# dwkim606/optimal_conv

Measured on AMD Instinct MI355X. Metric: homomorphic convs/sec (conv_then_pack + BN bias, k x k, batch B, N=2^16), higher is better.
Workload: dtype u64; 1 GPU; conv 3 3; ker_wid=3, batch=256, in_wid=16, logN=16, moduli=ckks.DefaultBootstrapParams[6] Q0,Q1 + P=0x1fffffffffe00001, ciphertexts_per_launch_set=4, contexts_per_gpu=4, chunk_nodes=512

## Files before the change

### optimal_conv_amd/csrc/hc_arith.h

```cpp
#pragma once
#include <stdint.h>

#if defined(__HIPCC__) || defined(HC_EMU)
#define HC_HD __host__ __device__ __forceinline__
#else
#define HC_HD inline
#endif

typedef uint64_t u64;
typedef unsigned int u32;
typedef unsigned __int128 u128;

HC_HD u64 hc_mulhi(u64 a, u64 b) {
#if defined(__HIP_DEVICE_COMPILE__)
    return __umul64hi(a, b);
#else
    return (u64)(((u128)a * b) >> 64);
#endif
}

HC_HD u64 hc_mul_shoup_lazy(u64 x, u64 w, u64 wp, u64 q) {
    u64 hi = hc_mulhi(x, wp);
    return x * w - hi * q;
}
HC_HD double hc_f64_mulmod(double x, double w, double wq, double q) {
#pragma clang fp contract(off)
    const double h = x * w;
    const double l = __builtin_fma(x, w, -h);
    const double k = __builtin_rint(x * wq);
    const double r = __builtin_fma(-k, q, h);
    return r + l;
}
HC_HD double hc_f64_reduce(double u, double q, double qinv) {
#pragma clang fp contract(off)
    return __builtin_fma(-__builtin_rint(u * qinv), q, u);
}
HC_HD double hc_u2d(u64 x) { return __builtin_bit_cast(double, x); }
HC_HD u64 hc_d2u(double x) { return __builtin_bit_cast(u64, x); }
HC_HD double hc_f64_from_u(u64 x) { return hc_u2d(x | 0x4330000000000000ull) - 4503599627370496.0; }
HC_HD u64 hc_f64_to_u_plus(double v, u64 base) { return (hc_d2u(v + 6755399441055744.0) & 0x000FFFFFFFFFFFFFull) + (base - 0x0008000000000000ull); }

HC_HD u64 hc_shoup_companion(u64 w, u64 q) {
    u64 r = w, quo = 0;
    for (int i = 0; i < 64; i++) {
        r <<= 1; quo <<= 1;
        if (r >= q) { r -= q; quo |= 1; }
    }
    return quo;
}
HC_HD u64 hc_csub(u64 x, u64 q) { return x >= q ? x - q : x; }

HC_HD u64 hc_mulhi_lo2(u64 x, u64 p) {
    const u32 x0 = (u32)x, x1 = (u32)(x >> 32), p0 = (u32)p, p1 = (u32)(p >> 32);
    return (u64)x1 * p1 + (((u64)x0 * p1) >> 32) + (((u64)x1 * p0) >> 32);
}
HC_HD u64 hc_opaque_uniform(u64 v) {
#if defined(__HIP_DEVICE_COMPILE__)
    u64 r;
    asm("; uniform constant kept opaque" : "=s"(r) : "0"(v));
    return r;
#else
    return v;
#endif
}
struct HcQ { u64 q, nq, q4, nq4, nq2; };
HC_HD HcQ hc_q(u64 q) {
    HcQ Q; Q.q = q; Q.nq = hc_opaque_uniform(0 - q); Q.q4 = 4 * q; Q.nq4 = hc_opaque_uniform(0 - 4 * q); Q.nq2 = hc_opaque_uniform(0 - 2 * q);
    return Q;
}
HC_HD u64 hc_shoup4(u64 x, u64 w, u64 wp, const HcQ &Q) { return x * w + hc_mulhi_lo2(x, wp) * Q.nq; }
HC_HD u64 hc_fold(u64 x, u64 nb) { const u64 t = x + nb; return (int)(u32)(t >> 32) < 0 ? x : t; }
HC_HD u64 hc_canon4(u64 x, const HcQ &Q) { return hc_fold(hc_fold(x, Q.nq2), Q.nq); }
HC_HD u64 hc_canon8(u64 x, const HcQ &Q) { return hc_canon4(hc_fold(x, Q.nq4), Q); }
HC_HD u64 hc_reduce64(u64 x, u64 mu, const HcQ &Q) { return hc_canon4(x + hc_mulhi_lo2(x, mu) * Q.nq, Q); }
HC_HD u64 hc_mul_shoup(u64 x, u64 w, u64 wp, u64 q) { return hc_csub(hc_mul_shoup_lazy(x, w, wp, q), q); }

HC_HD u64 hc_mont(u64 a, u64 b, u64 q, u64 qinv) {
    u128 m = (u128)a * b;
    u64 lo = (u64)m, hi = (u64)(m >> 64);
    u64 h = hc_mulhi(lo * qinv, q);
    u64 r = hi - h;
    return hi < h ? r + q : r;
}
HC_HD u64 hc_mont_redc(u128 T, u64 q, u64 qinv) {
    const u64 lo = (u64)T, hi = (u64)(T >> 64);
    const u64 h = hc_mulhi(lo * qinv, q);
    const u64 r = hi - h;
    return hi < h ? r + q : r;
}
HC_HD u64 hc_addmod(u64 a, u64 b, u64 q) { return hc_csub(a + b, q); }
HC_HD u64 hc_submod(u64 a, u64 b, u64 q) { return a >= b ? a - b : a + q - b; }

struct HcMod {
    u64 q;
    u64 qinv;
    u64 r2;
    u64 ninv, ninv_s;
    u64 mu;
    u64 row32;
};
```

### optimal_conv_amd/csrc/hc_kernels.h

```cpp
#pragma once
#include "hc_arith.h"

#define HC_TPB 256
#ifndef HC_MIN_WAVES
#define HC_MIN_WAVES 4
#endif
#define HC_ROWS_LDS 4096
#define HC_COLS_LDS 4096

struct __attribute__((aligned(16))) HcTw { u64 w, ws; };

#define HC_SMALL_Q(q) ((q) < (1ull << 31))
template <bool B> struct HcBool { static constexpr bool value = B; };
template <int V> struct HcInt { static constexpr int value = V; };
#define HC_COUNT_DISPATCH(n, body) do { switch (n) { case 1: body(HcInt<1>{}); break; case 2: body(HcInt<2>{}); break; case 3: body(HcInt<3>{}); break; case 4: body(HcInt<4>{}); break; \
    case 5: body(HcInt<5>{}); break; case 6: body(HcInt<6>{}); break; case 7: body(HcInt<7>{}); break; case 8: body(HcInt<8>{}); break; default: break; } } while (0)
#define HC_LD(S32, rowptr, j) ((S32) ? hc_ld32(rowptr, j) : (rowptr)[j])
#define HC_ST(S32, rowptr, j, v) do { if (S32) hc_st32(rowptr, j, v); else (rowptr)[j] = (v); } while (0)
#define HC_ROW_DISPATCH(row32, body) do { if (row32) body(HcBool<true>{}); else body(HcBool<false>{}); } while (0)
__device__ __forceinline__ u64 hc_ld32(const u64 *row, size_t j) { return (u64)reinterpret_cast<const u32 *>(row)[j]; }
__device__ __forceinline__ void hc_st32(u64 *row, size_t j, u64 v) { reinterpret_cast<u32 *>(row)[j] = (u32)v; }
struct __attribute__((packed, aligned(4))) HcU64A4 { u64 v; };
__device__ __forceinline__ u64 hc_ldp(const u64 *row, size_t j, bool row32) {
    return reinterpret_cast<const HcU64A4 *>(reinterpret_cast<const char *>(row) + (j << (row32 ? 2 : 3)))->v & (row32 ? 0xFFFFFFFFull : ~0ull);
}
struct HcTwTab {
    const HcTw *rowsA;
    const HcTw *rowsB;
    const HcTw *colsA;
    const HcTw *colsB;
    HcTw ninv;
    HcTw w_last_ninv;
};

struct __attribute__((aligned(8))) HcTw32 { u32 w, ws; };
struct HcTwTab32 { const HcTw32 *rowsA, *rowsB, *colsA, *colsB; };

enum { HC_FM_FREE = 1, HC_FM_ALT = 2 };
template <int FM, class TW>
__device__ __forceinline__ void hc_ct_round(u64 (&e)[16], const TW &tw, const HcQ &Q) {
#pragma unroll
    for (int s = 0; s < 4; s++) {
        const int half = 8 >> s;
#pragma unroll
        for (int g = 0; g < (1 << s); g++) {
            const HcTw w = tw((1 << s) - 1 + g);
#pragma unroll
            for (int k = 0; k < half; k++) {
                const int a = g * 2 * half + k, b = a + half;
                u64 X = e[a];
                if (FM == HC_FM_ALT) X = hc_fold(X, Q.nq4);
                const u64 T = hc_shoup4(e[b], w.w, w.ws, Q);
                e[a] = X + T;
                e[b] = (X + Q.q4) - T;
            }
        }
    }
}
template <int FM>
__device__ __forceinline__ u64 hc_fwd_canon(u64 x, const HcQ &Q, u64 mu) {
    if (FM == HC_FM_FREE) return hc_reduce64(x, mu, Q);
    return hc_canon8(x, Q);
}
template <bool LAST, class TW>
__device__ __forceinline__ void hc_gs_round(u64 (&e)[16], const TW &tw, const HcQ &Q, HcTw ninv, HcTw w_last) {
#pragma unroll
    for (int s = 0; s < 4; s++) {
        const int dist = 1 << s;
#pragma unroll
        for (int g = 0; g < (8 >> s); g++) {
            HcTw w = tw((8 >> s) - 1 + g);
            if (LAST && s == 3) w = w_last;
#pragma unroll
            for (int k = 0; k < dist; k++) {
                const int a = g * 2 * dist + k, b = a + dist;
                const u64 X = e[a], Y = e[b], u = X + Y, d = (X + Q.q4) - Y;
                if (LAST && s == 3) e[a] = hc_shoup4(u, ninv.w, ninv.ws, Q);
                else e[a] = hc_fold(u, Q.nq4);
                e[b] = hc_shoup4(d, w.w, w.ws, Q);
            }
        }
    }
}

struct HcF64Mod { double q, qinv; };
template <bool LAST, class TW>
__device__ __forceinline__ void hc_gs_round_f64(double (&e)[16], const TW &tw, HcF64Mod m, HcTw ninv, HcTw w_last) {
#pragma unroll
    for (int s = 0; s < 4; s++) {
        const int dist = 1 << s;
#pragma unroll
        for (int g = 0; g < (8 >> s); g++) {
            HcTw w = tw((8 >> s) - 1 + g);
            if (LAST && s == 3) w = w_last;
            const double ww = hc_u2d(w.w), wq = hc_u2d(w.ws);
#pragma unroll
            for (int k = 0; k < dist; k++) {
                const int a = g * 2 * dist + k, b = a + dist;
                const double X = e[a], Y = e[b], u = X + Y, d = X - Y;
                if (LAST && s == 3) e[a] = hc_f64_mulmod(u, hc_u2d(ninv.w), hc_u2d(ninv.ws), m.q);
                else e[a] = (s & 1) ? hc_f64_reduce(u, m.q, m.qinv) : u;
                e[b] = hc_f64_mulmod(d, ww, wq, m.q);
            }
        }
    }
}

#ifndef HC_ROWS_WAVE_SYNC
#define HC_ROWS_WAVE_SYNC 1
#endif
#if defined(HC_EMU) || !HC_ROWS_WAVE_SYNC
#define HC_ROW_SYNC() __syncthreads()
#else
#define HC_ROW_SYNC() do { __builtin_amdgcn_fence(__ATOMIC_RELEASE, "wavefront"); __builtin_amdgcn_wave_barrier(); __builtin_amdgcn_fence(__ATOMIC_ACQUIRE, "wavefront"); } while (0)
#endif
__device__ __forceinline__ int hc_rows_lds(int rloc, int col) {
    return rloc * 256 + ((col & 0xF0) ^ ((rloc & 1) << 4)) + ((col & 15) ^ ((col >> 5) & 7) ^ ((rloc & 1) << 3));
}
__device__ __forceinline__ int hc_cols_lds(int row, int c) { return ((row ^ ((row >> 4) & 1)) << 4) + c; }

#if defined(__HIP_DEVICE_COMPILE__)
typedef const HcTw __attribute__((address_space(1))) *HcTwGlobalPtr;
typedef const HcTw __attribute__((address_space(4))) *HcTwConstPtr;
#define HC_TW_LOAD(p, i) (*((HcTwGlobalPtr)(p) + (i)))
#define HC_TW_LOADK(p, i) (*((HcTwConstPtr)(p) + (i)))
#else
#define HC_TW_LOAD(p, i) ((p)[i])
#define HC_TW_LOADK(p, i) ((p)[i])
#endif
template <class T>
__device__ __forceinline__ T hc_const_copy(const T *p) {
    T r;
#if defined(__HIP_DEVICE_COMPILE__)
    static_assert(sizeof(T) % 8 == 0 && alignof(T) >= 8, "hc_const_copy: whole 8-byte words");
    typedef const u64 __attribute__((address_space(4))) *W;
    const W src = (W)(const void *)p; u64 *dst = reinterpret_cast<u64 *>(&r);
#pragma unroll
    for (unsigned i = 0; i < sizeof(T) / 8; i++) dst[i] = src[i];
#else
    r = *p;
#endif
    return r;
}
template <bool KC = false> struct HcRowsTwA { const HcTw *p; __device__ __forceinline__ HcTw operator()(int slot) const { if (KC) return HC_TW_LOADK(p, slot); else return HC_TW_LOAD(p, slot); } };
#ifndef HC_DBG_TWB_FIXED
#define HC_DBG_TWB_FIXED 0
#endif
template <bool KC = false> struct HcRowsTwB { const HcTw *p; __device__ __forceinline__ HcTw operator()(int slot) const { if (HC_DBG_TWB_FIXED) slot = 0; if (KC) return HC_TW_LOADK(p, slot * 16); else return HC_TW_LOAD(p, slot * 16); } };

template <int FM, bool KC = false>
__device__ __forceinline__ void hc_rows_fwd(u64 (&e)[16], u64 *lds, const HcTwTab &T, int row, int rloc, int tid, const HcQ &Q) {
    hc_ct_round<FM>(e, HcRowsTwA<KC>{T.rowsA + row * 16}, Q);
#pragma unroll
    for (int hi = 0; hi < 16; hi++) lds[hc_rows_lds(rloc, hi * 16 + tid)] = e[hi];
    HC_ROW_SYNC();
#pragma unroll
    for (int lo = 0; lo < 16; lo++) e[lo] = lds[hc_rows_lds(rloc, tid * 16 + lo)];
    hc_ct_round<FM>(e, HcRowsTwB<KC>{T.rowsB + row * 256 + tid}, Q);
}
template <bool KC = false>
__device__ __forceinline__ void hc_rows_inv(u64 (&e)[16], u64 *lds, const HcTwTab &T, int row, int rloc, int tid, const HcQ &Q) {
    hc_gs_round<false>(e, HcRowsTwB<KC>{T.rowsB + row * 256 + tid}, Q, T.ninv, T.ninv);
#pragma unroll
    for (int lo = 0; lo < 16; lo++) lds[hc_rows_lds(rloc, tid * 16 + lo)] = e[lo];
    HC_ROW_SYNC();
#pragma unroll
    for (int hi = 0; hi < 16; hi++) e[hi] = lds[hc_rows_lds(rloc, hi * 16 + tid)];
    hc_gs_round<false>(e, HcRowsTwA<KC>{T.rowsA + row * 16}, Q, T.ninv, T.ninv);
}
template <int FM, bool KC = false>
__device__ __forceinline__ void hc_cols_fwd(u64 (&e)[16], u64 *lds, const HcTwTab &T, int c, int tid, const HcQ &Q) {
    hc_ct_round<FM>(e, HcRowsTwA<KC>{T.colsA}, Q);
#pragma unroll
    for (int hi = 0; hi < 16; hi++) lds[hc_cols_lds(hi * 16 + tid, c)] = e[hi];
    __syncthreads();
#pragma unroll
    for (int lo = 0; lo < 16; lo++) e[lo] = lds[hc_cols_lds(tid * 16 + lo, c)];
    hc_ct_round<FM>(e, HcRowsTwB<KC>{T.colsB + tid}, Q);
}
template <bool SCALE = true, bool KC = false>
__device__ __forceinline__ void hc_cols_inv(u64 (&e)[16], u64 *lds, const HcTwTab &T, int c, int tid, const HcQ &Q) {
    hc_gs_round<false>(e, HcRowsTwB<KC>{T.colsB + tid}, Q, T.ninv, T.ninv);
#pragma unroll
    for (int lo = 0; lo < 16; lo++) lds[hc_cols_lds(tid * 16 + lo, c)] = e[lo];
    __syncthreads();
#pragma unroll
    for (int hi = 0; hi < 16; hi++) e[hi] = lds[hc_cols_lds(hi * 16 + tid, c)];
    hc_gs_round<SCALE>(e, HcRowsTwA<KC>{T.colsA}, Q, T.ninv, T.w_last_ninv);
}

__device__ __forceinline__ void hc_rows_inv_f64(double (&e)[16], u64 *lds, const HcTwTab &T, int row, int rloc, int tid, HcF64Mod m) {
    hc_gs_round_f64<false>(e, HcRowsTwB<false>{T.rowsB + row * 256 + tid}, m, T.ninv, T.ninv);
#pragma unroll
    for (int lo = 0; lo < 16; lo++) lds[hc_rows_lds(rloc, tid * 16 + lo)] = hc_d2u(e[lo]);
    HC_ROW_SYNC();
#pragma unroll
    for (int hi = 0; hi < 16; hi++) e[hi] = hc_u2d(lds[hc_rows_lds(rloc, hi * 16 + tid)]);
    hc_gs_round_f64<false>(e, HcRowsTwA<false>{T.rowsA + row * 16}, m, T.ninv, T.ninv);
}
__device__ __forceinline__ void hc_cols_inv_f64(double (&e)[16], u64 *lds, const HcTwTab &T, int c, int tid, HcF64Mod m) {
    hc_gs_round_f64<false>(e, HcRowsTwB<false>{T.colsB + tid}, m, T.ninv, T.ninv);
#pragma unroll
    for (int lo = 0; lo < 16; lo++) lds[hc_cols_lds(tid * 16 + lo, c)] = hc_d2u(e[lo]);
    __syncthreads();
#pragma unroll
    for (int hi = 0; hi < 16; hi++) e[hi] = hc_u2d(lds[hc_cols_lds(hi * 16 + tid, c)]);
    hc_gs_round_f64<true>(e, HcRowsTwA<false>{T.colsA}, m, T.ninv, T.w_last_ninv);
}

__device__ __forceinline__ void hc_rows_lin_to_lo(u64 (&e)[16], u64 *lds, int t, int rloc, int tid) {
#pragma unroll
    for (int k = 0; k < 16; k++) lds[hc_rows_lds(k, t)] = e[k];
    __syncthreads();
#pragma unroll
    for (int lo = 0; lo < 16; lo++) e[lo] = lds[hc_rows_lds(rloc, tid * 16 + lo)];
}
__device__ __forceinline__ void hc_rows_lo_to_lin(u64 (&e)[16], u64 *lds, int t, int rloc, int tid) {
#pragma unroll
    for (int lo = 0; lo < 16; lo++) lds[hc_rows_lds(rloc, tid * 16 + lo)] = e[lo];
    __syncthreads();
#pragma unroll
    for (int k = 0; k < 16; k++) e[k] = lds[hc_rows_lds(k, t)];
}

#ifndef HC_MM_LDS32
#define HC_MM_LDS32 1
#endif
#ifndef HC_MM_WAVES
#define HC_MM_WAVES 7
#endif
#ifndef HC_MM_WAVES_EXT
#define HC_MM_WAVES_EXT 5
#endif
#ifndef HC_CV_LDS32
#define HC_CV_LDS32 1
#endif
#if HC_CV_LDS32
typedef u32 hc_cvc_lds_t;
#else
typedef u64 hc_cvc_lds_t;
#endif
typedef u64 hc_cvr_lds_t;
#if HC_MM_LDS32
typedef u32 hc_mm_lds_t;
#else
typedef u64 hc_mm_lds_t;
#endif
__device__ __forceinline__ int hc_rows_lds32(int rloc, int col) {
    return rloc * 256 + ((col & 0xF0) ^ ((rloc & 1) << 4) ^ ((rloc & 2) << 4)) + ((col & 15) ^ ((col >> 5) & 7) ^ ((rloc & 1) << 3));
}
__device__ __forceinline__ int hc_cols_lds32(int row, int c) { return ((row ^ ((row >> 4) & 3)) << 4) + c; }
template <class WA, class RA, class SY>
__device__ __forceinline__ void hc_xchg32(u64 (&e)[16], u32 *lds, WA wa, RA ra, SY sync) {
    u32 lo[16];
#pragma unroll
    for (int i = 0; i < 16; i++) lds[wa(i)] = (u32)e[i];
    sync();
#pragma unroll
    for (int i = 0; i < 16; i++) lo[i] = lds[ra(i)];
    sync();
#pragma unroll
    for (int i = 0; i < 16; i++) lds[wa(i)] = (u32)(e[i] >> 32);
    sync();
#pragma unroll
    for (int i = 0; i < 16; i++) e[i] = ((u64)lds[ra(i)] << 32) | lo[i];
}
template <int FM, bool KC = false>
__device__ __forceinline__ void hc_rows_fwd(u64 (&e)[16], u32 *lds, const HcTwTab &T, int row, int rloc, int tid, const HcQ &Q) {
    hc_ct_round<FM>(e, HcRowsTwA<KC>{T.rowsA + row * 16}, Q);
    hc_xchg32(e, lds, [&](int hi) { return hc_rows_lds32(rloc, hi * 16 + tid); }, [&](int lo) { return hc_rows_lds32(rloc, tid * 16 + lo); }, [] { HC_ROW_SYNC(); });
    hc_ct_round<FM>(e, HcRowsTwB<KC>{T.rowsB + row * 256 + tid}, Q);
}
template <bool KC = false>
__device__ __forceinline__ void hc_rows_inv(u64 (&e)[16], u32 *lds, const HcTwTab &T, int row, int rloc, int tid, const HcQ &Q) {
    hc_gs_round<false>(e, HcRowsTwB<KC>{T.rowsB + row * 256 + tid}, Q, T.ninv, T.ninv);
    hc_xchg32(e, lds, [&](int lo) { return hc_rows_lds32(rloc, tid * 16 + lo); }, [&](int hi) { return hc_rows_lds32(rloc, hi * 16 + tid); }, [] { HC_ROW_SYNC(); });
    hc_gs_round<false>(e, HcRowsTwA<KC>{T.rowsA + row * 16}, Q, T.ninv, T.ninv);
}
template <int FM, bool KC = false>
__device__ __forceinline__ void hc_cols_fwd(u64 (&e)[16], u32 *lds, const HcTwTab &T, int c, int tid, const HcQ &Q) {
    hc_ct_round<FM>(e, HcRowsTwA<KC>{T.colsA}, Q);
    hc_xchg32(e, lds, [&](int hi) { return hc_cols_lds32(hi * 16 + tid, c); }, [&](int lo) { return hc_cols_lds32(tid * 16 + lo, c); }, [] { __syncthreads(); });
    hc_ct_round<FM>(e, HcRowsTwB<KC>{T.colsB + tid}, Q);
}
template <bool SCALE = true, bool KC = false>
__device__ __forceinline__ void hc_cols_inv(u64 (&e)[16], u32 *lds, const HcTwTab &T, int c, int tid, const HcQ &Q) {
    hc_gs_round<false>(e, HcRowsTwB<KC>{T.colsB + tid}, Q, T.ninv, T.ninv);
    hc_xchg32(e, lds, [&](int lo) { return hc_cols_lds32(tid * 16 + lo, c); }, [&](int hi) { return hc_cols_lds32(hi * 16 + tid, c); }, [] { __syncthreads(); });
    hc_gs_round<SCALE>(e, HcRowsTwA<KC>{T.colsA}, Q, T.ninv, T.w_last_ninv);
}
template <class WA, class RA, class SY>
__device__ __forceinline__ void hc_xchg32_f64(double (&f)[16], u32 *lds, WA wa, RA ra, SY sync) {
    u64 b[16];
#pragma unroll
    for (int i = 0; i < 16; i++) b[i] = hc_d2u(f[i]);
    hc_xchg32(b, lds, wa, ra, sync);
#pragma unroll
    for (int i = 0; i < 16; i++) f[i] = hc_u2d(b[i]);
}
// ... 390 lines not shown
#define HC_JOB_FAST 0
#endif
#if HC_JOB_FAST
#define HC_JOB blockIdx.x
#define HC_TILE blockIdx.y
#define HC_NJOBS gridDim.x
#else
#define HC_JOB blockIdx.y
#define HC_TILE blockIdx.x
#define HC_NJOBS gridDim.y
#endif
#define HC_FREE_OFF 72
#ifndef HC_W_A1
#define HC_W_A1 4
#endif
#ifndef HC_W_A2
#define HC_W_A2 4
#endif
#ifndef HC_W_A3
#define HC_W_A3 4
#endif
#ifndef HC_W_B1
#define HC_W_B1 4
#endif
#ifndef HC_W_B2
#define HC_W_B2 1
#endif
#ifndef HC_W_B3
#define HC_W_B3 4
#endif
#ifndef HC_W_B4
#define HC_W_B4 1
#endif
struct HcLoopA {
    const HcTw *ctc;
    HcPtrs ker;
    u64 *tmp;
    u64 *cts;
    int i0, norm;
    int slot0, slot_step;
    size_t cts_stride;
    int njobs;
    HcMod m0, m1;
    HcTw q1inv;
    u64 h, negh0;
};
#ifndef HC_A_WAVES
#define HC_A_WAVES 4
#endif
template <int F64>
__global__ __launch_bounds__(HC_TPB, HC_W_A1) void hc_k_a1(HcLoopA A, HcTwTab T1inv) {
    __shared__ hc_cvr_lds_t lds[HC_ROWS_LDS];
    const int t = threadIdx.x, tid = t & 15, rloc = t >> 4, row = HC_TILE * 16 + rloc;
    const int job = HC_JOB, p = job & 1, i = A.i0 + (job >> 1) * A.norm, z = blockIdx.z;
    const HcTw *__restrict__ c = A.ctc + ((size_t)z * 4 + (size_t)p * 2 + 1) * 65536;
    const u64 *__restrict__ k = A.ker.p[z] + ((size_t)i * 2 + 1) * 65536;
    const HcQ Q = hc_q(A.m1.q);
    u64 e[16];
#pragma unroll
    for (int kk = 0; kk < 16; kk++) {
        const size_t off = (size_t)(HC_TILE * 16 + kk) * 256 + t;
        const HcTw cw = c[off];
        e[kk] = hc_shoup4(k[off], cw.w, cw.ws, Q);
    }
    u64 *o = A.tmp + ((size_t)z * A.njobs + job) * 65536 + (size_t)row * 256;
    hc_rows_lin_to_lo(e, lds, t, rloc, tid);
    HC_ROW_SYNC();
    if (F64) {
        const HcF64Mod m{(double)A.m1.q, 1.0 / (double)A.m1.q};
        double f[16];
#pragma unroll
        for (int kk = 0; kk < 16; kk++) f[kk] = hc_f64_reduce(hc_f64_from_u(e[kk]), m.q, m.qinv);
        hc_rows_inv_f64(f, lds, T1inv, row, rloc, tid, m);
#pragma unroll
        for (int hi = 0; hi < 16; hi++) o[hi * 16 + tid] = hc_d2u(f[hi]);
    } else {
        hc_rows_inv(e, lds, T1inv, row, rloc, tid, Q);
#pragma unroll
        for (int hi = 0; hi < 16; hi++) o[hi * 16 + tid] = e[hi];
    }
}
template <int FM, int F64>
__global__ __launch_bounds__(HC_TPB, HC_W_A2) void hc_k_a2(HcLoopA A, HcTwTab T1inv, HcTwTab T0fwd) {
    __shared__ hc_cvc_lds_t lds[HC_COLS_LDS];
    const int t = threadIdx.x, c = t & 15, tid = t >> 4;
    u64 *base = A.tmp + (size_t)HC_JOB * 65536 + HC_TILE * 16 + c;
    const HcQ Q0 = hc_q(A.m0.q);
    u64 e[16];
#pragma unroll
    for (int lo = 0; lo < 16; lo++) e[lo] = base[(size_t)(tid * 16 + lo) * 256];
    if (F64) {
        const double q1 = (double)A.m1.q, hh = (double)A.h;
        const HcF64Mod m{q1, 1.0 / q1};
        double f[16];
#pragma unroll
        for (int lo = 0; lo < 16; lo++) f[lo] = hc_u2d(e[lo]);
        hc_cols_inv_f64(f, lds, T1inv, c, tid, m);
#pragma unroll
        for (int hi = 0; hi < 16; hi++) {
            double v = f[hi];
            v = v > hh ? v - q1 : (v < -hh ? v + q1 : v);
            e[hi] = hc_f64_to_u_plus(v, A.m0.q);
        }
    } else {
        const HcQ Q1 = hc_q(A.m1.q);
        hc_cols_inv(e, lds, T1inv, c, tid, Q1);
#pragma unroll
        for (int hi = 0; hi < 16; hi++) {
            const u64 v = hc_csub(hc_canon4(e[hi], Q1) + A.h, A.m1.q);
            e[hi] = hc_reduce64(v + A.negh0, A.m0.mu, Q0);
        }
    }
    __syncthreads();
    hc_cols_fwd<FM>(e, lds, T0fwd, c, tid, Q0);
#pragma unroll
    for (int lo = 0; lo < 16; lo++) base[(size_t)(tid * 16 + lo) * 256] = e[lo];
}
template <int FM>
__global__ __launch_bounds__(HC_TPB, HC_W_A3) void hc_k_a3(HcLoopA A, HcTwTab T0fwd) {
    __shared__ hc_cvr_lds_t lds[HC_ROWS_LDS];
    const int t = threadIdx.x, tid = t & 15, rloc = t >> 4, row = HC_TILE * 16 + rloc;
    const int job = HC_JOB, p = job & 1, i = A.i0 + (job >> 1) * A.norm, z = blockIdx.z;
    const u64 *__restrict__ in = A.tmp + ((size_t)z * A.njobs + job) * 65536 + (size_t)row * 256;
    const HcTw *__restrict__ c = A.ctc + ((size_t)z * 4 + (size_t)p * 2) * 65536 + (size_t)HC_TILE * 4096 + t;
    const u64 *__restrict__ k = A.ker.p[z] + ((size_t)i * 2) * 65536 + (size_t)HC_TILE * 4096 + t;
    u64 *__restrict__ o = A.cts + (size_t)z * A.cts_stride + ((size_t)(A.slot0 + (job >> 1) * A.slot_step) * 2 + p) * 65536 + (size_t)HC_TILE * 4096 + t;
    const HcQ Q = hc_q(A.m0.q);
    u64 e[16], a0[16];
#pragma unroll
    for (int hi = 0; hi < 16; hi++) e[hi] = in[hi * 16 + tid];
#pragma unroll
    for (int kk = 0; kk < 16; kk++) a0[kk] = k[kk * 256];
#pragma unroll
    for (int kk = 0; kk < 16; kk++) { const HcTw cw = c[kk * 256]; a0[kk] = hc_shoup4(a0[kk], cw.w, cw.ws, Q); }
    hc_rows_fwd<FM>(e, lds, T0fwd, row, rloc, tid, Q);
    HC_ROW_SYNC();
    hc_rows_lo_to_lin(e, lds, t, rloc, tid);
#pragma unroll
    for (int kk = 0; kk < 16; kk++) {
        const u64 d = FM == HC_FM_FREE ? a0[kk] + HC_FREE_OFF * Q.q - e[kk] : a0[kk] + Q.q - hc_canon8(e[kk], Q);
        o[kk * 256] = hc_canon4(hc_shoup4(d, A.q1inv.w, A.q1inv.ws, Q), Q);
    }
}

struct HcLoopB {
    const u64 *src;
    u64 *dst;
    u64 *tmpC;
    u64 *tmpE;
    u64 *tmpT;
    const HcTw *idx;
    const HcTw *evkQ;
    const HcTw *evkP;
    int n0, step, norm;
    int nodes;
    size_t src_stride, dst_stride;
    HcMod m0, mp;
    HcTw pmodq;
    HcTw pinv;
    u64 mu0;
    u64 vthresh;
    u32 gal;
};
__global__ __launch_bounds__(HC_TPB, HC_W_B1) void hc_k_b1(HcLoopB B, HcTwTab T0inv) {
    __shared__ hc_cvr_lds_t lds[HC_ROWS_LDS];
    const int t = threadIdx.x, tid = t & 15, rloc = t >> 4, row = HC_TILE * 16 + rloc;
    const int job = HC_JOB, z = job / B.nodes, node = job - z * B.nodes, i = (B.n0 + node) * B.norm;
    const size_t tile = (size_t)HC_TILE * 4096 + t;
    const u64 *__restrict__ y1 = B.src + (size_t)z * B.src_stride + ((size_t)i * 2 + 1) * 65536 + tile;
    const u64 *__restrict__ x1 = B.src + (size_t)z * B.src_stride + ((size_t)(i + B.step) * 2 + 1) * 65536 + tile;
    const HcTw *__restrict__ idx = B.idx + tile;
    const HcQ Q = hc_q(B.m0.q);
    u64 e[16], yy[16];
#pragma unroll
    for (int kk = 0; kk < 16; kk++) { e[kk] = x1[kk * 256]; yy[kk] = y1[kk * 256]; }
#pragma unroll
    for (int kk = 0; kk < 16; kk++) {
        const HcTw I = idx[kk * 256];
        e[kk] = hc_fold(yy[kk] + Q.q4 - hc_shoup4(e[kk], I.w, I.ws, Q), Q.nq4);
    }
    if (B.tmpT != nullptr) {
        u64 *__restrict__ tt = B.tmpT + (size_t)job * 65536 + tile;
#pragma unroll
        for (int kk = 0; kk < 16; kk++) tt[kk * 256] = e[kk];
    }
    hc_rows_lin_to_lo(e, lds, t, rloc, tid);
    HC_ROW_SYNC();
    hc_rows_inv(e, lds, T0inv, row, rloc, tid, Q);
    u64 *__restrict__ o = B.tmpC + (size_t)job * 65536 + (size_t)row * 256;
#pragma unroll
    for (int hi = 0; hi < 16; hi++) o[hi * 16 + tid] = e[hi];
}
template <int FMP>
__global__ __launch_bounds__(HC_TPB, HC_W_B2) void hc_k_b2(HcLoopB B, HcTwTab T0inv, HcTwTab TPfwd) {
    __shared__ hc_cvc_lds_t lds[HC_COLS_LDS];
    const int t = threadIdx.x, c = t & 15, tid = t >> 4;
    u64 *base = B.tmpC + (size_t)HC_JOB * 65536 + HC_TILE * 16 + c;
    const HcQ Q0 = hc_q(B.m0.q), QP = hc_q(B.mp.q);
    u64 e[16];
#pragma unroll
    for (int lo = 0; lo < 16; lo++) e[lo] = base[(size_t)(tid * 16 + lo) * 256];
    hc_cols_inv(e, lds, T0inv, c, tid, Q0);
#pragma unroll
    for (int hi = 0; hi < 16; hi++) e[hi] = hc_canon4(e[hi], Q0);
    __syncthreads();
    hc_cols_fwd<FMP>(e, lds, TPfwd, c, tid, QP);
#pragma unroll
    for (int lo = 0; lo < 16; lo++) base[(size_t)(tid * 16 + lo) * 256] = e[lo];
}
template <int FMP>
__global__ __launch_bounds__(HC_TPB, HC_W_B3) void hc_k_b3(HcLoopB B, HcTwTab TPfwd, HcTwTab TPinv) {
    __shared__ hc_cvr_lds_t lds[HC_ROWS_LDS];
    const int t = threadIdx.x, tid = t & 15, rloc = t >> 4, row = HC_TILE * 16 + rloc;
    const int node = HC_JOB;
    const u64 *in = B.tmpC + (size_t)node * 65536 + (size_t)row * 256;
    const HcQ Q = hc_q(B.mp.q);
    u64 cp[16], e[16];
#pragma unroll
    for (int hi = 0; hi < 16; hi++) cp[hi] = in[hi * 16 + tid];
    hc_rows_fwd<FMP>(cp, lds, TPfwd, row, rloc, tid, Q);
#pragma unroll
    for (int k = 0; k < 2; k++) {
        const HcTw *__restrict__ ev = B.evkP + (size_t)k * 65536 + (size_t)HC_TILE * 4096 + t;
#pragma unroll
        for (int lo = 0; lo < 16; lo++) {
            const HcTw w = ev[lo * 256];
            e[lo] = hc_shoup4(cp[lo], w.w, w.ws, Q);
        }
        HC_ROW_SYNC();
        hc_rows_inv(e, lds, TPinv, row, rloc, tid, Q);
        u64 *o = B.tmpE + ((size_t)node * 2 + k) * 65536 + (size_t)row * 256;
#pragma unroll
        for (int hi = 0; hi < 16; hi++) o[hi * 16 + tid] = e[hi];
    }
}
template <int FM>
__global__ __launch_bounds__(HC_TPB, HC_W_B4) void hc_k_b4(HcLoopB B, HcTwTab TPinv, HcTwTab T0fwd) {
    __shared__ hc_cvc_lds_t lds[HC_COLS_LDS];
    const int t = threadIdx.x, c = t & 15, tid = t >> 4;
    u64 *base = B.tmpE + (size_t)HC_JOB * 65536 + HC_TILE * 16 + c;
    const HcQ QP = hc_q(B.mp.q), Q = hc_q(B.m0.q);
    u64 e[16];
#pragma unroll
    for (int lo = 0; lo < 16; lo++) e[lo] = base[(size_t)(tid * 16 + lo) * 256];
    hc_cols_inv<false>(e, lds, TPinv, c, tid, QP);
#pragma unroll
    for (int hi = 0; hi < 16; hi++) {
        const u64 yv = hc_canon4(e[hi], QP);
        u64 r = hc_shoup4(yv, B.pinv.w, B.pinv.ws, Q);
        if (yv >= B.vthresh) r += Q.q - 1;
        e[hi] = r;
    }
    __syncthreads();
    hc_cols_fwd<FM>(e, lds, T0fwd, c, tid, Q);
#pragma unroll
    for (int lo = 0; lo < 16; lo++) base[(size_t)(tid * 16 + lo) * 256] = e[lo];
}
template <int FM, int K0>
__device__ __forceinline__ void hc_b5_terms(u64 Y, u64 T, HcTw K, u64 X, HcTw I, const HcQ &Q, u64 &t1, u64 &f) {
    const u64 q = Q.q;
    u64 g = hc_shoup4(T, K.w, K.ws, Q);
    if (FM != HC_FM_FREE) g = hc_canon4(g, Q);
    if (K0) {
        u64 m = hc_shoup4(X, I.w, I.ws, Q);
        if (FM == HC_FM_FREE) { t1 = Y + m; f = Y + Q.q4 - m + g; }
        else { m = hc_canon4(m, Q); t1 = hc_addmod(Y, m, q); f = hc_addmod(hc_submod(Y, m, q), g, q); }
    } else {
        if (FM == HC_FM_FREE) t1 = Y + Y + Q.q4 - T;
        else t1 = hc_addmod(Y, hc_submod(Y, hc_canon4(T, Q), q), q);
        f = g;
    }
}
template <int FM>
__global__ __launch_bounds__(HC_TPB, 3) void hc_k_b5(HcLoopB B, HcTwTab T0fwd, HcPtrs biases, HcPtrs outs) {
    __shared__ u64 lds[HC_ROWS_LDS];
    const int t = threadIdx.x, tid = t & 15, rloc = t >> 4, row = HC_TILE * 16 + rloc;
    const int job = HC_JOB, zn = job >> 1, k = job & 1, z = zn / B.nodes, node = zn - z * B.nodes, i = (B.n0 + node) * B.norm;
    const HcQ Q = hc_q(B.m0.q);
    const u64 q = Q.q;
    const size_t tile = (size_t)HC_TILE * 4096 + t;
    const u64 *__restrict__ in = B.tmpE + (size_t)job * 65536 + (size_t)row * 256;
    const u64 *__restrict__ yk = B.src + (size_t)z * B.src_stride + ((size_t)i * 2 + k) * 65536 + tile;
    const u64 *__restrict__ xk = B.src + (size_t)z * B.src_stride + ((size_t)(i + B.step) * 2 + k) * 65536 + tile;
    const u64 *__restrict__ tc1 = B.tmpT + (size_t)zn * 65536 + tile;
    const HcTw *__restrict__ idx = B.idx + tile;
    const HcTw *__restrict__ evk = B.evkQ + (size_t)k * 65536 + tile;
    u64 *__restrict__ o = (outs.p[z] != nullptr ? const_cast<u64 *>(outs.p[z]) + (size_t)k * 65536 : B.dst + (size_t)z * B.dst_stride + ((size_t)i * 2 + k) * 65536) + tile;
    const u64 *__restrict__ bias = (k == 0 && biases.p[z] != nullptr) ? biases.p[z] + tile : nullptr;
    u64 e[16];
#pragma unroll
    for (int hi = 0; hi < 16; hi++) e[hi] = in[hi * 16 + tid];
    hc_rows_fwd<FM>(e, lds, T0fwd, row, rloc, tid, Q);
    HC_ROW_SYNC();
    hc_rows_lo_to_lin(e, lds, t, rloc, tid);
    __syncthreads();
    {
        u64 t1[16];
#pragma unroll
        for (int b = 0; b < 16; b += 4) {
            u64 Y[4], T[4], X[4]; HcTw K[4], I[4];
#pragma unroll
            for (int j = 0; j < 4; j++) {
                const int off = (b + j) * 256;
                Y[j] = yk[off]; K[j] = evk[off]; T[j] = tc1[off];
                if (k == 0) { X[j] = xk[off]; I[j] = idx[off]; } else { X[j] = 0; I[j] = K[j]; }
            }
#pragma unroll
            for (int j = 0; j < 4; j++) {
                const int kk = b + j;
                u64 f;
                if (k == 0) hc_b5_terms<FM, 1>(Y[j], T[j], K[j], X[j], I[j], Q, t1[kk], f);
                else hc_b5_terms<FM, 0>(Y[j], T[j], K[j], X[j], I[j], Q, t1[kk], f);
                if (bias != nullptr) t1[kk] = FM == HC_FM_FREE ? t1[kk] + bias[kk * 256] : hc_addmod(t1[kk], bias[kk * 256], q);
                lds[hc_rows_lds(kk, t)] = FM == HC_FM_FREE ? f + HC_FREE_OFF * q - e[kk] : hc_submod(f, hc_canon8(e[kk], Q), q);
            }
        }
        __syncthreads();
#pragma unroll
        for (int kk = 0; kk < 16; kk++) {
            const u32 srcidx = hc_perm_src((u32)((HC_TILE * 16 + kk) * 256 + t), B.gal);
            const u64 d = lds[hc_rows_lds((int)((srcidx >> 8) & 15), (int)(srcidx & 255))];
            o[kk * 256] = FM == HC_FM_FREE ? hc_reduce64(t1[kk] + d, B.m0.mu, Q) : hc_addmod(t1[kk], d, q);
        }
    }
}

#ifndef HC_B5_ROWS
#define HC_B5_ROWS 2
#endif
#ifndef HC_B5M_UNROLL
#define HC_B5M_UNROLL 2
#endif
#ifndef HC_B5M_WAVES
#define HC_B5M_WAVES 3
#endif
#ifndef HC_B5M_PIPE
#define HC_B5M_PIPE 0
#endif
#define HC_PRAGMA_(x) _Pragma(#x)
#define HC_UNROLL_N(n) HC_PRAGMA_(unroll n)
template <int FM>
__global__ __launch_bounds__(HC_TPB, HC_B5M_WAVES) void hc_k_b5m(HcLoopB B, HcTwTab T0fwd, HcPtrs biases, HcPtrs outs) {
    __shared__ u64 lds[HC_ROWS_LDS];
    const int t = threadIdx.x, tid = t & 15, rloc = t >> 4, row = HC_TILE * 16 + rloc;
    const int zn = HC_JOB, z = zn / B.nodes, node = zn - z * B.nodes, i = (B.n0 + node) * B.norm;
    const HcQ Q = hc_q(B.m0.q);
    const u64 q = Q.q;
    const size_t tile = (size_t)HC_TILE * 4096 + t;
    const u64 *__restrict__ ys = B.src + (size_t)z * B.src_stride + (size_t)i * 2 * 65536 + tile;
    const u64 *__restrict__ xs = B.src + (size_t)z * B.src_stride + (size_t)(i + B.step) * 2 * 65536 + tile;
    const HcTw *__restrict__ idx = B.idx + tile;
    const HcTw *__restrict__ evk = B.evkQ + tile;
    u64 *__restrict__ o = (outs.p[z] != nullptr ? const_cast<u64 *>(outs.p[z]) : B.dst + (size_t)z * B.dst_stride + (size_t)i * 2 * 65536) + tile;
    const u64 *__restrict__ bias = biases.p[z] != nullptr ? biases.p[z] + tile : nullptr;
    u64 e[16], T[16];
#if HC_B5M_PIPE
    HC_UNROLL_N(HC_B5M_UNROLL)
    for (int k = 1; k >= 0; k--) {
        const u64 *__restrict__ in = B.tmpE + ((size_t)zn * 2 + k) * 65536 + (size_t)row * 256;
#pragma unroll
        for (int hi = 0; hi < 16; hi++) e[hi] = in[hi * 16 + tid];
        u64 Yn[HC_B5_ROWS], Xn[HC_B5_ROWS], bn[HC_B5_ROWS]; HcTw Kn[HC_B5_ROWS], In[HC_B5_ROWS];
#pragma unroll
        for (int j = 0; j < HC_B5_ROWS; j++) {
            const int off = j * 256;
            Yn[j] = ys[(size_t)k * 65536 + off]; Xn[j] = xs[(size_t)k * 65536 + off]; In[j] = idx[off]; Kn[j] = evk[(size_t)k * 65536 + off];
            bn[j] = (k == 0 && bias != nullptr) ? bias[off] : 0;
        }
        if (k == 0) __syncthreads();
        hc_rows_fwd<FM>(e, lds, T0fwd, row, rloc, tid, Q);
        HC_ROW_SYNC();
        hc_rows_lo_to_lin(e, lds, t, rloc, tid);
        __syncthreads();
#pragma unroll
        for (int b = 0; b < 16; b += HC_B5_ROWS) {
            u64 Y[HC_B5_ROWS], X[HC_B5_ROWS], t1[HC_B5_ROWS], bs[HC_B5_ROWS]; HcTw K[HC_B5_ROWS], I[HC_B5_ROWS];
#pragma unroll
            for (int j = 0; j < HC_B5_ROWS; j++) { Y[j] = Yn[j]; X[j] = Xn[j]; I[j] = In[j]; K[j] = Kn[j]; bs[j] = bn[j]; }
            if (b + HC_B5_ROWS < 16) {
#pragma unroll
                for (int j = 0; j < HC_B5_ROWS; j++) {
                    const int off = (b + HC_B5_ROWS + j) * 256;
                    Yn[j] = ys[(size_t)k * 65536 + off]; Xn[j] = xs[(size_t)k * 65536 + off]; In[j] = idx[off]; Kn[j] = evk[(size_t)k * 65536 + off];
                    bn[j] = (k == 0 && bias != nullptr) ? bias[off] : 0;
                }
            }
#pragma unroll
            for (int j = 0; j < HC_B5_ROWS; j++) {
                const int kk = b + j;
                u64 m = hc_shoup4(X[j], I[j].w, I[j].ws, Q), f;
                if (k == 1) T[kk] = hc_fold(Y[j] + Q.q4 - m, Q.nq4);
                u64 g = hc_shoup4(T[kk], K[j].w, K[j].ws, Q);
                if (FM == HC_FM_FREE) {
                    t1[j] = Y[j] + m + bs[j];
                    f = (k == 0 ? Y[j] + Q.q4 - m + g : g) + HC_FREE_OFF * q - e[kk];
                } else {
                    m = hc_canon4(m, Q); g = hc_canon4(g, Q);
                    t1[j] = hc_addmod(hc_addmod(Y[j], m, q), bs[j], q);
                    f = hc_submod(k == 0 ? hc_addmod(hc_submod(Y[j], m, q), g, q) : g, hc_canon8(e[kk], Q), q);
                }
                lds[hc_rows_lds(kk, t)] = f;
            }
            __syncthreads();
#pragma unroll
            for (int j = 0; j < HC_B5_ROWS; j++) {
                const int kk = b + j;
                const u32 srcidx = hc_perm_src((u32)((HC_TILE * 16 + kk) * 256 + t), B.gal);
                const u64 d = lds[hc_rows_lds(kk, (int)(srcidx & 255))];
                o[(size_t)k * 65536 + kk * 256] = FM == HC_FM_FREE ? hc_reduce64(t1[j] + d, B.m0.mu, Q) : hc_addmod(t1[j], d, q);
            }
        }
    }
#else
    HC_UNROLL_N(HC_B5M_UNROLL)
    for (int k = 1; k >= 0; k--) {
        const u64 *__restrict__ in = B.tmpE + ((size_t)zn * 2 + k) * 65536 + (size_t)row * 256;
#pragma unroll
        for (int hi = 0; hi < 16; hi++) e[hi] = in[hi * 16 + tid];
        if (k == 0) __syncthreads();
        hc_rows_fwd<FM>(e, lds, T0fwd, row, rloc, tid, Q);
        HC_ROW_SYNC();
        hc_rows_lo_to_lin(e, lds, t, rloc, tid);
        __syncthreads();
#pragma unroll
        for (int b = 0; b < 16; b += HC_B5_ROWS) {
            u64 Y[HC_B5_ROWS], X[HC_B5_ROWS], t1[HC_B5_ROWS], bs[HC_B5_ROWS]; HcTw K[HC_B5_ROWS], I[HC_B5_ROWS];
#pragma unroll
            for (int j = 0; j < HC_B5_ROWS; j++) {
                const int off = (b + j) * 256;
                Y[j] = ys[(size_t)k * 65536 + off]; X[j] = xs[(size_t)k * 65536 + off]; I[j] = idx[off]; K[j] = evk[(size_t)k * 65536 + off];
                bs[j] = (k == 0 && bias != nullptr) ? bias[off] : 0;
            }
#pragma unroll
            for (int j = 0; j < HC_B5_ROWS; j++) {
                const int kk = b + j;
                u64 m = hc_shoup4(X[j], I[j].w, I[j].ws, Q), f;
                if (k == 1) T[kk] = hc_fold(Y[j] + Q.q4 - m, Q.nq4);
                u64 g = hc_shoup4(T[kk], K[j].w, K[j].ws, Q);
                if (FM == HC_FM_FREE) {
                    t1[j] = Y[j] + m + bs[j];
                    f = (k == 0 ? Y[j] + Q.q4 - m + g : g) + HC_FREE_OFF * q - e[kk];
                } else {
                    m = hc_canon4(m, Q); g = hc_canon4(g, Q);
                    t1[j] = hc_addmod(hc_addmod(Y[j], m, q), bs[j], q);
                    f = hc_submod(k == 0 ? hc_addmod(hc_submod(Y[j], m, q), g, q) : g, hc_canon8(e[kk], Q), q);
                }
                lds[hc_rows_lds(kk, t)] = f;
            }
            __syncthreads();
#pragma unroll
            for (int j = 0; j < HC_B5_ROWS; j++) {
                const int kk = b + j;
                const u32 srcidx = hc_perm_src((u32)((HC_TILE * 16 + kk) * 256 + t), B.gal);
                const u64 d = lds[hc_rows_lds(kk, (int)(srcidx & 255))];
                o[(size_t)k * 65536 + kk * 256] = FM == HC_FM_FREE ? hc_reduce64(t1[j] + d, B.m0.mu, Q) : hc_addmod(t1[j], d, q);
            }
        }
    }
#endif
}

#ifndef HC_B5M_LOADER
#define HC_B5M_LOADER 0
#endif
#if HC_B5M_LOADER && !defined(HC_EMU)
#ifndef HC_LD_RING
#define HC_LD_RING 4
#endif
#ifndef HC_LD_AUX
#define HC_LD_AUX 0
#endif
#define HC_LD_SLOT 1536
#define HC_LD_TPB (HC_TPB + 64)
typedef const void __attribute__((address_space(1))) *HcGlobalVoidPtr;
typedef void __attribute__((address_space(3))) *HcLdsVoidPtr;
__device__ __forceinline__ void hc_wait_vmcnt(int n) {
#define HC_VMC(k) case k: asm volatile("s_waitcnt vmcnt(" #k ")" ::: "memory"); break;
    switch (n) { HC_VMC(0) HC_VMC(12) HC_VMC(24) HC_VMC(36) HC_VMC(48) HC_VMC(60) default: asm volatile("s_waitcnt vmcnt(0)" ::: "memory"); break; }
#undef HC_VMC
}
__device__ __forceinline__ void hc_ld_row(u64 *ring, int slot, const u64 *ys, const u64 *xs, const HcTw *idx, const HcTw *evk, int k, int kk, int lane) {
    u64 *s = ring + slot * HC_LD_SLOT;
    const u64 *y = ys + (size_t)k * 65536 + kk * 256 + lane * 2, *x = xs + (size_t)k * 65536 + kk * 256 + lane * 2;
    const HcTw *I = idx + kk * 256 + lane, *K = evk + (size_t)k * 65536 + kk * 256 + lane;
#pragma unroll
    for (int h = 0; h < 2; h++) {
        __builtin_amdgcn_global_load_lds((HcGlobalVoidPtr)(y + h * 128), (HcLdsVoidPtr)(s + h * 128), 16, 0, HC_LD_AUX);
        __builtin_amdgcn_global_load_lds((HcGlobalVoidPtr)(x + h * 128), (HcLdsVoidPtr)(s + 256 + h * 128), 16, 0, HC_LD_AUX);
    }
#pragma unroll
    for (int h = 0; h < 4; h++) {
        __builtin_amdgcn_global_load_lds((HcGlobalVoidPtr)(I + h * 64), (HcLdsVoidPtr)(s + 512 + h * 128), 16, 0, 0);
        __builtin_amdgcn_global_load_lds((HcGlobalVoidPtr)(K + h * 64), (HcLdsVoidPtr)(s + 1024 + h * 128), 16, 0, 0);
    }
}
__device__ __forceinline__ void hc_ld_rows(int g0, int g1, u64 *ring, const u64 *ys, const u64 *xs, const HcTw *idx, const HcTw *evk, int lane) {
#pragma unroll
    for (int g = g0; g < g1; g++)
        if (g < 32) hc_ld_row(ring, g % HC_LD_RING, ys, xs, idx, evk, g < 16 ? 1 : 0, g & 15, lane);
}
constexpr int hc_ld_min(int a, int b) { return a < b ? a : b; }
template <int FM>
__global__ __launch_bounds__(HC_LD_TPB, 3) void hc_k_b5m_ld(HcLoopB B, HcTwTab T0fwd, HcPtrs biases, HcPtrs outs) {
    __shared__ u64 lds[HC_ROWS_LDS + HC_LD_RING * HC_LD_SLOT];
    u64 *ring = lds + HC_ROWS_LDS;
    constexpr int R = HC_B5_ROWS, S = HC_LD_RING, NBAT = 16 / R;
    static_assert(S >= 2 * R && S % R == 0 && (S - R) * 12 <= 60, "ring: at least two row batches, a whole number of them, and a vmcnt that fits its 6-bit field");
    const int zn = HC_JOB, z = zn / B.nodes, node = zn - z * B.nodes, i = (B.n0 + node) * B.norm;
    const size_t tile0 = (size_t)HC_TILE * 4096;
    const u64 *__restrict__ ys0 = B.src + (size_t)z * B.src_stride + (size_t)i * 2 * 65536 + tile0;
    const u64 *__restrict__ xs0 = B.src + (size_t)z * B.src_stride + (size_t)(i + B.step) * 2 * 65536 + tile0;
    if (threadIdx.x >= HC_TPB) {
        const int lane = threadIdx.x - HC_TPB;
        const HcTw *idx0 = B.idx + tile0, *evk0 = B.evkQ + tile0;
        hc_ld_rows(0, S, ring, ys0, xs0, idx0, evk0, lane);
#pragma unroll
        for (int k = 1; k >= 0; k--) {
            const int gb0 = (1 - k) * NBAT;
            if (k == 0) __builtin_amdgcn_s_barrier();
            __builtin_amdgcn_s_barrier();
            hc_wait_vmcnt((hc_ld_min(gb0 * R + S, 32) - (gb0 + 1) * R) * 12);
            __builtin_amdgcn_s_barrier();
#pragma unroll
            for (int b = 0; b < NBAT; b++) {
                const int gb = gb0 + b, left = hc_ld_min(gb * R + S, 32) - (gb + 2) * R;
                if (b + 1 < NBAT) hc_wait_vmcnt(left < 0 ? 0 : left * 12);
                __builtin_amdgcn_s_barrier();
                hc_ld_rows(gb * R + S, gb * R + S + R, ring, ys0, xs0, idx0, evk0, lane);
            }
        }
        return;
    }
    const int t = threadIdx.x, tid = t & 15, rloc = t >> 4, row = HC_TILE * 16 + rloc;
    const HcQ Q = hc_q(B.m0.q);
    const u64 q = Q.q;
    u64 *__restrict__ o = (outs.p[z] != nullptr ? const_cast<u64 *>(outs.p[z]) : B.dst + (size_t)z * B.dst_stride + (size_t)i * 2 * 65536) + tile0 + t;
    const u64 *__restrict__ bias = biases.p[z] != nullptr ? biases.p[z] + tile0 + t : nullptr;
    u64 e[16], T[16];
    HC_UNROLL_N(HC_B5M_UNROLL)
    for (int k = 1; k >= 0; k--) {
        const u64 *__restrict__ in = B.tmpE + ((size_t)zn * 2 + k) * 65536 + (size_t)row * 256;
#pragma unroll
        for (int hi = 0; hi < 16; hi++) e[hi] = in[hi * 16 + tid];
        if (k == 0) __syncthreads();
        hc_rows_fwd<FM>(e, lds, T0fwd, row, rloc, tid, Q);
        HC_ROW_SYNC();
        hc_rows_lo_to_lin(e, lds, t, rloc, tid);
        __syncthreads();
        auto epilogue = [&](auto HB) {
            constexpr bool HASB = decltype(HB)::value;
#pragma unroll
            for (int b = 0; b < 16; b += R) {
                u64 Y[R], X[R], t1[R], bs[R]; HcTw K[R], I[R];
#pragma unroll
                for (int j = 0; j < R; j++) {
                    const u64 *s = ring + (((1 - k) * 16 + b + j) % S) * HC_LD_SLOT;
                    Y[j] = s[t]; X[j] = s[256 + t]; I[j] = *reinterpret_cast<const HcTw *>(s + 512 + 2 * t); K[j] = *reinterpret_cast<const HcTw *>(s + 1024 + 2 * t);
                    bs[j] = HASB ? bias[(b + j) * 256] : 0;
                }
#pragma unroll
                for (int j = 0; j < R; j++) {
                    const int kk = b + j;
                    u64 m = hc_shoup4(X[j], I[j].w, I[j].ws, Q), f;
                    if (k == 1) T[kk] = hc_fold(Y[j] + Q.q4 - m, Q.nq4);
                    u64 g = hc_shoup4(T[kk], K[j].w, K[j].ws, Q);
                    if (FM == HC_FM_FREE) {
                        t1[j] = Y[j] + m + bs[j];
                        f = (k == 0 ? Y[j] + Q.q4 - m + g : g) + HC_FREE_OFF * q - e[kk];
                    } else {
                        m = hc_canon4(m, Q); g = hc_canon4(g, Q);
                        t1[j] = hc_addmod(hc_addmod(Y[j], m, q), bs[j], q);
                        f = hc_submod(k == 0 ? hc_addmod(hc_submod(Y[j], m, q), g, q) : g, hc_canon8(e[kk], Q), q);
                    }
                    lds[hc_rows_lds(kk, t)] = f;
                }
                __syncthreads();
#pragma unroll
                for (int j = 0; j < R; j++) {
                    const int kk = b + j;
                    const u32 srcidx = hc_perm_src((u32)((HC_TILE * 16 + kk) * 256 + t), B.gal);
                    const u64 d = lds[hc_rows_lds(kk, (int)(srcidx & 255))];
                    o[(size_t)k * 65536 + kk * 256] = FM == HC_FM_FREE ? hc_reduce64(t1[j] + d, B.m0.mu, Q) : hc_addmod(t1[j], d, q);
                }
            }
        };
        if (k == 0 && bias != nullptr) epilogue(HcBool<true>{}); else epilogue(HcBool<false>{});
    }
}
#endif

#define HC_STPB 256
#define HC_STILES 64
#define HC_S_LDS 1024
template <bool ROWS> __device__ __forceinline__ int hc_s_addr(int line, int x) { return ROWS ? line * 256 + x : x * 4 + line; }
__device__ __forceinline__ int hc_s_pos(int u, int lo) { return (u & ((1 << lo) - 1)) | ((u >> lo) << (lo + 2)); }
template <bool ROWS, int D> __device__ __forceinline__ HcTw hc_s_tw_fwd(const HcTwTab &T, int x, int gline) {
    if (D >= 16) { constexpr int s = D == 128 ? 0 : D == 64 ? 1 : D == 32 ? 2 : 3; const int slot = (1 << s) - 1 + (x >> (8 - s)); return ROWS ? T.rowsA[gline * 16 + slot] : T.colsA[slot]; }
    constexpr int s = D == 8 ? 0 : D == 4 ? 1 : D == 2 ? 2 : 3; const int slot = (1 << s) - 1 + ((x & 15) >> (4 - s));
    return ROWS ? T.rowsB[gline * 256 + slot * 16 + (x >> 4)] : T.colsB[slot * 16 + (x >> 4)];
}
template <bool ROWS, int D> __device__ __forceinline__ HcTw hc_s_tw_inv(const HcTwTab &T, int x, int gline) {
    if (D <= 8) { constexpr int s = D == 1 ? 0 : D == 2 ? 1 : D == 4 ? 2 : 3; const int slot = (8 >> s) - 1 + ((x & 15) >> (s + 1)); return ROWS ? T.rowsB[gline * 256 + slot * 16 + (x >> 4)] : T.colsB[slot * 16 + (x >> 4)]; }
    constexpr int s = D == 16 ? 0 : D == 32 ? 1 : D == 64 ? 2 : 3; const int slot = (8 >> s) - 1 + (x >> (5 + s));
    return ROWS ? T.rowsA[gline * 16 + slot] : T.colsA[slot];
}
__device__ __forceinline__ void hc_s_bf_fwd(u64 &X, u64 &Y, HcTw w, const HcQ &Q) { const u64 x = hc_fold(X, Q.nq4), t = hc_shoup4(Y, w.w, w.ws, Q); X = x + t; Y = (x + Q.q4) - t; }
__device__ __forceinline__ void hc_s_bf_inv(u64 &X, u64 &Y, HcTw w, const HcQ &Q) { const u64 u = X + Y, d = (X + Q.q4) - Y; X = hc_fold(u, Q.nq4); Y = hc_shoup4(d, w.w, w.ws, Q); }
template <bool ROWS> __device__ __forceinline__ void hc_s_tw_load_fwd(HcTw (&w)[12], const HcTwTab &T, int gline, int u) {
    { const int x0 = hc_s_pos(u, 6); w[0] = hc_s_tw_fwd<ROWS, 128>(T, x0, gline); w[1] = hc_s_tw_fwd<ROWS, 64>(T, x0, gline); w[2] = hc_s_tw_fwd<ROWS, 64>(T, x0 + 128, gline); }
    { const int x0 = hc_s_pos(u, 4); w[3] = hc_s_tw_fwd<ROWS, 32>(T, x0, gline); w[4] = hc_s_tw_fwd<ROWS, 16>(T, x0, gline); w[5] = hc_s_tw_fwd<ROWS, 16>(T, x0 + 32, gline); }
    { const int x0 = hc_s_pos(u, 2); w[6] = hc_s_tw_fwd<ROWS, 8>(T, x0, gline); w[7] = hc_s_tw_fwd<ROWS, 4>(T, x0, gline); w[8] = hc_s_tw_fwd<ROWS, 4>(T, x0 + 8, gline); }
    { const int x0 = hc_s_pos(u, 0); w[9] = hc_s_tw_fwd<ROWS, 2>(T, x0, gline); w[10] = hc_s_tw_fwd<ROWS, 1>(T, x0, gline); w[11] = hc_s_tw_fwd<ROWS, 1>(T, x0 + 2, gline); }
}
template <bool ROWS> __device__ __forceinline__ void hc_s_tw_load_inv(HcTw (&w)[12], const HcTwTab &T, int gline, int u) {
    { const int x0 = hc_s_pos(u, 0); w[0] = hc_s_tw_inv<ROWS, 1>(T, x0, gline); w[1] = hc_s_tw_inv<ROWS, 1>(T, x0 + 2, gline); w[2] = hc_s_tw_inv<ROWS, 2>(T, x0, gline); }
    { const int x0 = hc_s_pos(u, 2); w[3] = hc_s_tw_inv<ROWS, 4>(T, x0, gline); w[4] = hc_s_tw_inv<ROWS, 4>(T, x0 + 8, gline); w[5] = hc_s_tw_inv<ROWS, 8>(T, x0, gline); }
    { const int x0 = hc_s_pos(u, 4); w[6] = hc_s_tw_inv<ROWS, 16>(T, x0, gline); w[7] = hc_s_tw_inv<ROWS, 16>(T, x0 + 32, gline); w[8] = hc_s_tw_inv<ROWS, 32>(T, x0, gline); }
    { const int x0 = hc_s_pos(u, 6); w[9] = hc_s_tw_inv<ROWS, 64>(T, x0, gline); w[10] = hc_s_tw_inv<ROWS, 64>(T, x0 + 128, gline); w[11] = hc_s_tw_inv<ROWS, 128>(T, x0, gline); }
}
template <bool ROWS, int D> __device__ __forceinline__ void hc_s_round_fwd(u64 *lds, HcTw wa, HcTw wb, HcTw wc, int line, int u, const HcQ &Q) {
    constexpr int lo = D == 128 ? 6 : D == 32 ? 4 : D == 8 ? 2 : 0, H = D / 2;
    const int x0 = hc_s_pos(u, lo);
    u64 e0 = lds[hc_s_addr<ROWS>(line, x0)], e1 = lds[hc_s_addr<ROWS>(line, x0 + H)], e2 = lds[hc_s_addr<ROWS>(line, x0 + D)], e3 = lds[hc_s_addr<ROWS>(line, x0 + D + H)];
    hc_s_bf_fwd(e0, e2, wa, Q); hc_s_bf_fwd(e1, e3, wa, Q);
    hc_s_bf_fwd(e0, e1, wb, Q); hc_s_bf_fwd(e2, e3, wc, Q);
    lds[hc_s_addr<ROWS>(line, x0)] = e0; lds[hc_s_addr<ROWS>(line, x0 + H)] = e1; lds[hc_s_addr<ROWS>(line, x0 + D)] = e2; lds[hc_s_addr<ROWS>(line, x0 + D + H)] = e3;
}
template <bool ROWS, int D, bool SCALE_LAST> __device__ __forceinline__ void hc_s_round_inv(u64 *lds, const HcTwTab &T, HcTw wa, HcTw wb, HcTw wc, int line, int u, const HcQ &Q) {
    constexpr int lo = D == 1 ? 0 : D == 4 ? 2 : D == 16 ? 4 : 6, G = 2 * D;
    const int x0 = hc_s_pos(u, lo);
    u64 e0 = lds[hc_s_addr<ROWS>(line, x0)], e1 = lds[hc_s_addr<ROWS>(line, x0 + D)], e2 = lds[hc_s_addr<ROWS>(line, x0 + G)], e3 = lds[hc_s_addr<ROWS>(line, x0 + G + D)];
    hc_s_bf_inv(e0, e1, wa, Q); hc_s_bf_inv(e2, e3, wb, Q);
    if (SCALE_LAST) {
        const u64 ua = e0 + e2, da = (e0 + Q.q4) - e2, ub = e1 + e3, db = (e1 + Q.q4) - e3;
        e0 = hc_shoup4(ua, T.ninv.w, T.ninv.ws, Q); e2 = hc_shoup4(da, T.w_last_ninv.w, T.w_last_ninv.ws, Q);
        e1 = hc_shoup4(ub, T.ninv.w, T.ninv.ws, Q); e3 = hc_shoup4(db, T.w_last_ninv.w, T.w_last_ninv.ws, Q);
    } else { hc_s_bf_inv(e0, e2, wc, Q); hc_s_bf_inv(e1, e3, wc, Q); }
    lds[hc_s_addr<ROWS>(line, x0)] = e0; lds[hc_s_addr<ROWS>(line, x0 + D)] = e1; lds[hc_s_addr<ROWS>(line, x0 + G)] = e2; lds[hc_s_addr<ROWS>(line, x0 + G + D)] = e3;
}
template <bool ROWS> __device__ __forceinline__ void hc_s_sync() { if (ROWS) { HC_ROW_SYNC(); } else __syncthreads(); }
template <bool ROWS> __device__ __forceinline__ void hc_s_pass_fwd(u64 *lds, const HcTw (&w)[12], int line, int u, const HcQ &Q) {
    hc_s_round_fwd<ROWS, 128>(lds, w[0], w[1], w[2], line, u, Q); hc_s_sync<ROWS>();
    hc_s_round_fwd<ROWS, 32>(lds, w[3], w[4], w[5], line, u, Q); hc_s_sync<ROWS>();
    hc_s_round_fwd<ROWS, 8>(lds, w[6], w[7], w[8], line, u, Q); hc_s_sync<ROWS>();
    hc_s_round_fwd<ROWS, 2>(lds, w[9], w[10], w[11], line, u, Q); __syncthreads();
}
template <bool ROWS, bool SCALE> __device__ __forceinline__ void hc_s_pass_inv(u64 *lds, const HcTwTab &T, const HcTw (&w)[12], int line, int u, const HcQ &Q) {
    hc_s_round_inv<ROWS, 1, false>(lds, T, w[0], w[1], w[2], line, u, Q); hc_s_sync<ROWS>();
    hc_s_round_inv<ROWS, 4, false>(lds, T, w[3], w[4], w[5], line, u, Q); hc_s_sync<ROWS>();
    hc_s_round_inv<ROWS, 16, false>(lds, T, w[6], w[7], w[8], line, u, Q); hc_s_sync<ROWS>();
    hc_s_round_inv<ROWS, 64, SCALE>(lds, T, w[9], w[10], w[11], line, u, Q); __syncthreads();
}
#ifndef HC_S_REG_PASSES
#define HC_S_REG_PASSES 1
#endif
#if defined(HC_EMU)
template <int LB> __device__ __forceinline__ void hc_xswap(u64 &r0, u64 &r1) {
    __shared__ u64 xch[HC_STPB];
    const int t = threadIdx.x; const bool hi = (t >> LB) & 1;
    xch[t] = hi ? r0 : r1;
    __syncthreads();
    const u64 got = xch[t ^ (1 << LB)];
    __syncthreads();
    if (hi) r0 = got; else r1 = got;
}
#else
template <int LB> __device__ __forceinline__ void hc_xswap32(u32 &a, u32 &b) {
    if (LB == 5) { auto r = __builtin_amdgcn_permlane32_swap(a, b, false, false); a = r[0]; b = r[1]; }
    else if (LB == 4) { auto r = __builtin_amdgcn_permlane16_swap(a, b, false, false); a = r[0]; b = r[1]; }
    else if (LB == 3) { const u32 a0 = a; a = __builtin_amdgcn_update_dpp(a, b, 0x128, 0xF, 0xC, false); b = __builtin_amdgcn_update_dpp(b, a0, 0x128, 0xF, 0x3, false); }
    else if (LB == 2) { const u32 a0 = a; a = __builtin_amdgcn_update_dpp(a, b, 0x114, 0xF, 0xA, false); b = __builtin_amdgcn_update_dpp(b, a0, 0x104, 0xF, 0x5, false); }
    else {
        const bool hi = (threadIdx.x >> LB) & 1;
        const u32 give = hi ? a : b;
        const u32 got = LB == 1 ? __builtin_amdgcn_mov_dpp(give, 0x4E, 0xF, 0xF, true) : __builtin_amdgcn_mov_dpp(give, 0xB1, 0xF, 0xF, true);
        if (hi) a = got; else b = got;
    }
}
template <int LB> __device__ __forceinline__ void hc_xswap(u64 &r0, u64 &r1) {
    u32 a0 = (u32)r0, a1 = (u32)(r0 >> 32), b0 = (u32)r1, b1 = (u32)(r1 >> 32);
    hc_xswap32<LB>(a0, b0); hc_xswap32<LB>(a1, b1);
    r0 = ((u64)a1 << 32) | a0; r1 = ((u64)b1 << 32) | b0;
}
#endif
template <int HB> __device__ __forceinline__ void hc_s_transpose(u64 (&e)[4]) { hc_xswap<HB>(e[0], e[2]); hc_xswap<HB>(e[1], e[3]); hc_xswap<HB - 1>(e[0], e[1]); hc_xswap<HB - 1>(e[2], e[3]); }
__device__ __forceinline__ void hc_s_pass_fwd_reg(u64 (&e)[4], const HcTw (&w)[12], const HcQ &Q) {
    hc_s_bf_fwd(e[0], e[2], w[0], Q); hc_s_bf_fwd(e[1], e[3], w[0], Q); hc_s_bf_fwd(e[0], e[1], w[1], Q); hc_s_bf_fwd(e[2], e[3], w[2], Q);
    hc_s_transpose<5>(e);
    hc_s_bf_fwd(e[0], e[2], w[3], Q); hc_s_bf_fwd(e[1], e[3], w[3], Q); hc_s_bf_fwd(e[0], e[1], w[4], Q); hc_s_bf_fwd(e[2], e[3], w[5], Q);
    hc_s_transpose<3>(e);
    hc_s_bf_fwd(e[0], e[2], w[6], Q); hc_s_bf_fwd(e[1], e[3], w[6], Q); hc_s_bf_fwd(e[0], e[1], w[7], Q); hc_s_bf_fwd(e[2], e[3], w[8], Q);
    hc_s_transpose<1>(e);
    hc_s_bf_fwd(e[0], e[2], w[9], Q); hc_s_bf_fwd(e[1], e[3], w[9], Q); hc_s_bf_fwd(e[0], e[1], w[10], Q); hc_s_bf_fwd(e[2], e[3], w[11], Q);
}
__device__ __forceinline__ void hc_s_pass_inv_reg(u64 (&e)[4], const HcTw (&w)[12], const HcQ &Q) {
    hc_s_bf_inv(e[0], e[1], w[0], Q); hc_s_bf_inv(e[2], e[3], w[1], Q); hc_s_bf_inv(e[0], e[2], w[2], Q); hc_s_bf_inv(e[1], e[3], w[2], Q);
    hc_s_transpose<1>(e);
    hc_s_bf_inv(e[0], e[1], w[3], Q); hc_s_bf_inv(e[2], e[3], w[4], Q); hc_s_bf_inv(e[0], e[2], w[5], Q); hc_s_bf_inv(e[1], e[3], w[5], Q);
    hc_s_transpose<3>(e);
    hc_s_bf_inv(e[0], e[1], w[6], Q); hc_s_bf_inv(e[2], e[3], w[7], Q); hc_s_bf_inv(e[0], e[2], w[8], Q); hc_s_bf_inv(e[1], e[3], w[8], Q);
    hc_s_transpose<5>(e);
    hc_s_bf_inv(e[0], e[1], w[9], Q); hc_s_bf_inv(e[2], e[3], w[10], Q); hc_s_bf_inv(e[0], e[2], w[11], Q); hc_s_bf_inv(e[1], e[3], w[11], Q);
}
#define HC_S_ROWS_MAP const int t = threadIdx.x, line = t >> 6, u = t & 63, grow = HC_TILE * 4 + line
#define HC_S_CTILE ((int)((blockIdx.x & 7) * 8 + (blockIdx.x >> 3)))
#define HC_S_COLS_MAP const int t = threadIdx.x, line = t & 3, u = t >> 2

__global__ __launch_bounds__(HC_STPB) void hc_k_sb1(HcLoopB B, HcTwTab T0inv) {
    __shared__ u64 lds[HC_S_LDS];
    HC_S_ROWS_MAP;
    const int job = HC_JOB, z = job / B.nodes, node = job - z * B.nodes, i = (B.n0 + node) * B.norm;
    const size_t tile = (size_t)HC_TILE * 1024;
    const u64 *__restrict__ y1 = B.src + (size_t)z * B.src_stride + ((size_t)i * 2 + 1) * 65536 + tile;
    const u64 *__restrict__ x1 = B.src + (size_t)z * B.src_stride + ((size_t)(i + B.step) * 2 + 1) * 65536 + tile;
    const HcTw *__restrict__ idx = B.idx + tile;
    const HcQ Q = hc_q(B.m0.q);
    HcTw w[12]; hc_s_tw_load_inv<true>(w, T0inv, grow, u);
    u64 *__restrict__ o = B.tmpC + (size_t)job * 65536 + tile;
#if HC_S_REG_PASSES
    (void)lds;
    u64 e[4];
#pragma unroll
    for (int j = 0; j < 4; j++) {
        const int p = line * 256 + u * 4 + j; const HcTw I = idx[p];
        e[j] = hc_fold(y1[p] + Q.q4 - hc_shoup4(x1[p], I.w, I.ws, Q), Q.nq4);
    }
    hc_s_pass_inv_reg(e, w, Q);
#pragma unroll
    for (int j = 0; j < 4; j++) o[line * 256 + j * 64 + u] = e[j];
#else
#pragma unroll
    for (int k = 0; k < 4; k++) {
        const int p = k * 256 + t; const HcTw I = idx[p];
        lds[p] = hc_fold(y1[p] + Q.q4 - hc_shoup4(x1[p], I.w, I.ws, Q), Q.nq4);
    }
    __syncthreads();
    hc_s_pass_inv<true, false>(lds, T0inv, w, line, u, Q);
#pragma unroll
    for (int k = 0; k < 4; k++) o[k * 256 + t] = lds[k * 256 + t];
#endif
}
__global__ __launch_bounds__(HC_STPB) void hc_k_sb2(HcLoopB B, HcTwTab T0inv, HcTwTab TPfwd) {
// ... 19 lines not shown
    HC_S_ROWS_MAP;
    const int node = HC_JOB, k = blockIdx.z;
    const size_t tile = (size_t)HC_TILE * 1024;
    const u64 *in = B.tmpC + (size_t)node * 65536 + tile;
    const HcQ Q = hc_q(B.mp.q);
    HcTw w[12]; hc_s_tw_load_fwd<true>(w, TPfwd, grow, u);
    const HcTw *__restrict__ ev = B.evkP + (size_t)k * 65536;
#if HC_S_REG_PASSES
    {
        (void)lds;
        u64 e[4];
#pragma unroll
        for (int j = 0; j < 4; j++) e[j] = in[line * 256 + j * 64 + u];
        hc_s_pass_fwd_reg(e, w, Q);
        hc_s_tw_load_inv<true>(w, TPinv, grow, u);
#pragma unroll
        for (int j = 0; j < 4; j++) {
            const int R = grow, C = u * 4 + j;
            const HcTw kw = ev[((R >> 4) * 16 + (C & 15)) * 256 + (R & 15) * 16 + (C >> 4)];
            e[j] = hc_shoup4(e[j], kw.w, kw.ws, Q);
        }
        hc_s_pass_inv_reg(e, w, Q);
        u64 *o = B.tmpE + ((size_t)node * 2 + k) * 65536 + tile;
#pragma unroll
        for (int j = 0; j < 4; j++) o[line * 256 + j * 64 + u] = e[j];
        return;
    }
#endif
#pragma unroll
    for (int j = 0; j < 4; j++) lds[j * 256 + t] = in[j * 256 + t];
    __syncthreads();
    hc_s_pass_fwd<true>(lds, w, line, u, Q);
    hc_s_tw_load_inv<true>(w, TPinv, grow, u);
#pragma unroll
    for (int j = 0; j < 4; j++) {
        const int p = j * 256 + t, R = HC_TILE * 4 + (p >> 8), C = p & 255;
        const HcTw w = ev[((R >> 4) * 16 + (C & 15)) * 256 + (R & 15) * 16 + (C >> 4)];
        lds[p] = hc_shoup4(lds[p], w.w, w.ws, Q);
    }
    __syncthreads();
    hc_s_pass_inv<true, false>(lds, TPinv, w, line, u, Q);
    u64 *o = B.tmpE + ((size_t)node * 2 + k) * 65536 + tile;
#pragma unroll
    for (int j = 0; j < 4; j++) o[j * 256 + t] = lds[j * 256 + t];
}
__global__ __launch_bounds__(HC_STPB) void hc_k_sb4(HcLoopB B, HcTwTab TPinv, HcTwTab T0fwd) {
    __shared__ u64 lds[HC_S_LDS];
    HC_S_COLS_MAP;
    u64 *base = B.tmpE + (size_t)HC_JOB * 65536 + HC_S_CTILE * 4;
    const HcQ QP = hc_q(B.mp.q), Q = hc_q(B.m0.q);
    HcTw w[12]; hc_s_tw_load_inv<false>(w, TPinv, 0, u);
#pragma unroll
    for (int k = 0; k < 4; k++) { const int r = k * 64 + u; lds[r * 4 + line] = base[(size_t)r * 256 + line]; }
    __syncthreads();
    hc_s_pass_inv<false, false>(lds, TPinv, w, line, u, QP);
    hc_s_tw_load_fwd<false>(w, T0fwd, 0, u);
#pragma unroll
    for (int k = 0; k < 4; k++) {
        const int a = (k * 64 + u) * 4 + line;
        const u64 yv = hc_canon4(lds[a], QP);
        u64 r = hc_shoup4(yv, B.pinv.w, B.pinv.ws, Q);
        if (yv >= B.vthresh) r += Q.q - 1;
        lds[a] = r;
    }
    __syncthreads();
    hc_s_pass_fwd<false>(lds, w, line, u, Q);
#pragma unroll
    for (int k = 0; k < 4; k++) { const int r = k * 64 + u; base[(size_t)r * 256 + line] = lds[r * 4 + line]; }
}
__global__ __launch_bounds__(HC_STPB) void hc_k_sb5(HcLoopB B, HcTwTab T0fwd, HcPtrs biases, HcPtrs outs) {
    __shared__ u64 lds[HC_S_LDS];
    HC_S_ROWS_MAP;
    const int job = HC_JOB, zn = job >> 1, k = job & 1, z = zn / B.nodes, node = zn - z * B.nodes, i = (B.n0 + node) * B.norm;
    const HcQ Q = hc_q(B.m0.q);
    const size_t tile = (size_t)HC_TILE * 1024;
    const u64 *__restrict__ in = B.tmpE + (size_t)job * 65536 + tile;
    const u64 *__restrict__ ys = B.src + (size_t)z * B.src_stride + (size_t)i * 2 * 65536 + tile;
    const u64 *__restrict__ xs = B.src + (size_t)z * B.src_stride + (size_t)(i + B.step) * 2 * 65536 + tile;
    const HcTw *__restrict__ idx = B.idx + tile;
    const HcTw *__restrict__ evk = B.evkQ + (size_t)k * 65536 + tile;
    u64 *__restrict__ o = (outs.p[z] != nullptr ? const_cast<u64 *>(outs.p[z]) + (size_t)k * 65536 : B.dst + (size_t)z * B.dst_stride + ((size_t)i * 2 + k) * 65536) + tile;
    const u64 *__restrict__ bias = (k == 0 && biases.p[z] != nullptr) ? biases.p[z] + tile : nullptr;
    HcTw w[12]; hc_s_tw_load_fwd<true>(w, T0fwd, grow, u);
#if HC_S_REG_PASSES
    u64 e[4];
#pragma unroll
    for (int j = 0; j < 4; j++) e[j] = hc_reduce64(in[line * 256 + j * 64 + u], B.m0.mu, Q);
    hc_s_pass_fwd_reg(e, w, Q);
#else
#pragma unroll
    for (int j = 0; j < 4; j++) lds[j * 256 + t] = in[j * 256 + t];
    __syncthreads();
    hc_s_pass_fwd<true>(lds, w, line, u, Q);
#endif
    u64 t1[4];
#pragma unroll
    for (int j = 0; j < 4; j++) {
#if HC_S_REG_PASSES
        const int p = line * 256 + u * 4 + j;
        const u64 nraw = e[j];
#else
        const int p = j * 256 + t;
        const u64 nraw = lds[p];
#endif
        const HcTw I = idx[p], K = evk[p];
        const u64 y1 = ys[65536 + p], x1 = xs[65536 + p];
        const u64 T = hc_fold(y1 + Q.q4 - hc_shoup4(x1, I.w, I.ws, Q), Q.nq4);
        const u64 g = hc_canon4(hc_shoup4(T, K.w, K.ws, Q), Q);
        const u64 n = hc_canon8(nraw, Q);
        u64 f;
        if (k == 0) {
            const u64 y0 = ys[p], m = hc_canon4(hc_shoup4(xs[p], I.w, I.ws, Q), Q);
            t1[j] = hc_addmod(y0, m, Q.q);
            if (bias != nullptr) t1[j] = hc_addmod(t1[j], bias[p], Q.q);
            f = hc_addmod(hc_submod(y0, m, Q.q), g, Q.q);
        } else {
            t1[j] = hc_addmod(y1, hc_submod(y1, hc_canon4(T, Q), Q.q), Q.q);
            f = g;
        }
        lds[p] = hc_submod(f, n, Q.q);
    }
    __syncthreads();
#pragma unroll
    for (int j = 0; j < 4; j++) {
#if HC_S_REG_PASSES
        const int p = line * 256 + u * 4 + j;
#else
        const int p = j * 256 + t;
#endif
        const u32 srcidx = hc_perm_src((u32)(HC_TILE * 1024 + p), B.gal);
        o[p] = hc_addmod(t1[j], lds[srcidx & 1023], Q.q);
    }
}



struct HcBasisExt {
    int n;
    u64 s[8];
    HcTw inv[8];
    HcTw hat[8];
    HcTw smodt;
    u64 t, mu_t;
    u64 mu_s[8];
};
#ifndef HC_EXT_GROUP
#define HC_EXT_GROUP 4
#endif
#ifndef HC_EXT_FULL
#define HC_EXT_FULL 1
#endif
#ifndef HC_DBG_EXT_ONELOAD
#define HC_DBG_EXT_ONELOAD 0
#endif
#define HC_MAX_NP 5
template <int NS>
__device__ __forceinline__ u64 hc_basis_ext_sum(const u64 (&y)[NS + 1], const HcBasisExt &B, const HcQ &Q) {
    const int n = B.n;
    u64 v = 0;
#pragma unroll
    for (int i = 0; i <= NS; i++) if (i == n) v = y[i];
    if (n == 1) return hc_barrett64(y[0], B.t, B.mu_t);
    const u64 vs = (u64)(u32)v * B.smodt.w;
    if (B.t < (1ull << 58)) {
        u64 acc = 2 * Q.q4, hi = 0;
#pragma unroll
        for (int i = 0; i < NS; i++) if (i < n) { acc += y[i] * B.hat[i].w; hi += hc_mulhi_lo2(y[i], B.hat[i].ws); }
        return hc_reduce64(acc + hi * Q.nq - vs, B.mu_t, Q);
    }
    u64 acc = 0;
#pragma unroll
    for (int i = 0; i < NS; i++) if (i < n) acc = hc_fold(acc + hc_shoup4(y[i], B.hat[i].w, B.hat[i].ws, Q), Q.nq4);
    return hc_canon8(acc + Q.q4 - hc_fold(vs, Q.nq4), Q);
}
template <int NS>
__device__ __forceinline__ u64 hc_basis_ext_sum_full(const u64 (&y)[NS + 1], const HcBasisExt &B, const HcQ &Q) {
    const u64 vs = (u64)(u32)y[NS] * B.smodt.w;
    if (B.t < (1ull << 58)) {
        u64 acc = 2 * Q.q4, hi = 0;
#pragma unroll
        for (int i = 0; i < NS; i++) { acc += y[i] * B.hat[i].w; hi += hc_mulhi_lo2(y[i], B.hat[i].ws); }
        return hc_reduce64(acc + hi * Q.nq - vs, B.mu_t, Q);
    }
    u64 acc = 0;
#pragma unroll
    for (int i = 0; i < NS; i++) acc = hc_fold(acc + hc_shoup4(y[i], B.hat[i].w, B.hat[i].ws, Q), Q.nq4);
    return hc_canon8(acc + Q.q4 - hc_fold(vs, Q.nq4), Q);
}
template <int NS>
__device__ __forceinline__ void hc_basis_ext_tile(u64 (&e)[16], const u64 *yv, const HcBasisExt &B, int tid) {
    const int n = B.n; const HcQ Q = hc_q(B.t);
    if (HC_EXT_FULL && NS > 1 && n == NS) {
#pragma unroll
        for (int g0 = 0; g0 < 16; g0 += HC_EXT_GROUP) {
            u64 y[HC_EXT_GROUP][NS + 1];
#pragma unroll
            for (int g = 0; g < HC_EXT_GROUP; g++) {
                const u64 *p = yv + (size_t)((g0 + g) * 16 + tid) * 256;
#pragma unroll
                for (int i = 0; i <= NS; i++) y[g][i] = p[(size_t)(HC_DBG_EXT_ONELOAD ? 0 : i) * 65536];
            }
#pragma unroll
            for (int g = 0; g < HC_EXT_GROUP; g++) e[g0 + g] = hc_basis_ext_sum_full<NS>(y[g], B, Q);
        }
        return;
    }
#pragma unroll
    for (int g0 = 0; g0 < 16; g0 += HC_EXT_GROUP) {
        u64 y[HC_EXT_GROUP][NS + 1];
#pragma unroll
        for (int g = 0; g < HC_EXT_GROUP; g++) {
            const u64 *p = yv + (size_t)((g0 + g) * 16 + tid) * 256;
#pragma unroll
            for (int i = 0; i <= NS; i++) if (i <= n) y[g][i] = p[(size_t)i * 65536];
        }
#pragma unroll
        for (int g = 0; g < HC_EXT_GROUP; g++) e[g0 + g] = hc_basis_ext_sum<NS>(y[g], B, Q);
    }
}
template <int NS>
__device__ __forceinline__ u32 hc_basis_ext_sum32(const u64 (&y)[NS + 1], const u32 (&hat)[NS], u64 off, u32 smodt, u64 t, u64 mu_t) {
    u64 H = 0, L = off - (u64)(u32)y[NS] * (u64)smodt;
#pragma unroll
    for (int i = 0; i < NS; i += 2) {
        u64 pair = 0;
#pragma unroll
        for (int k = i; k < i + 2 && k < NS; k++) {
            H += (u64)(u32)(y[k] >> 32) * hat[k];
            pair += (u64)(u32)y[k] * hat[k];
        }
        H += pair >> 32; L += (u64)(u32)pair;
    }
    const u64 r1 = hc_barrett64(H, t, mu_t);
    return (u32)hc_barrett64((r1 << 32) + L, t, mu_t);
}
template <int NS>
__device__ __forceinline__ void hc_basis_ext_tile32(u32 (&e)[16], const u64 *yv, const HcBasisExt &B, int tid) {
    const int n = B.n;
    const u64 t = B.t, mu_t = B.mu_t;
    if (n == 1) {
#pragma unroll
        for (int g = 0; g < 16; g++) e[g] = (u32)hc_barrett64(yv[(size_t)(g * 16 + tid) * 256], t, mu_t);
        return;
    }
    u32 hat[NS]; size_t roff[NS + 1];
#pragma unroll
    for (int i = 0; i < NS; i++) hat[i] = i < n ? (u32)B.hat[i].w : 0u;
#pragma unroll
    for (int i = 0; i <= NS; i++) roff[i] = (size_t)(i < n ? i : n) * 65536;
    const u32 smodt = (u32)B.smodt.w; const u64 off = 8 * t;
#pragma unroll
    for (int g0 = 0; g0 < 16; g0 += HC_EXT_GROUP) {
        u64 y[HC_EXT_GROUP][NS + 1];
#pragma unroll
        for (int g = 0; g < HC_EXT_GROUP; g++) {
            const u64 *p = yv + (size_t)((g0 + g) * 16 + tid) * 256;
#pragma unroll
            for (int i = 0; i <= NS; i++) y[g][i] = p[HC_DBG_EXT_ONELOAD ? 0 : roff[i]];
        }
#pragma unroll
        for (int g = 0; g < HC_EXT_GROUP; g++) e[g0 + g] = hc_basis_ext_sum32<NS>(y[g], hat, off, smodt, t, mu_t);
    }
}
struct HcRowMod { HcTwTab fwd, inv; u64 q, mu;
                  HcTwTab32 fwd32, inv32;
                  u64 s32; };
struct HcMm { const HcRowMod *M; int nl, nq, skip_lo, skip_hi; size_t zs_in, zs_out; int z_alpha; int nz; size_t is_in, is_out;
              int xcd, nzn;
              int out_gap;
              int pk_in, pk_out, pk_epi;
              int gap_lo, gap_len;

              int lift_level; const HcMod *mods; const HcBasisExt *ext_bs; int ext_rows;
              const u64 *lift_t; size_t lift_t_zs, lift_t_is; const HcTw *lift_pmul;
              const u64 *epi_x; size_t epi_x_zs, epi_x_is; const HcTw *epi_mul; const u64 *epi_add; size_t epi_add_zs, epi_add_is; const HcTw *epi_add_mul; };
__device__ __forceinline__ bool hc_mm_skip(const HcMm &A, int y, int zi) {
    if (A.z_alpha > 0) { const int lo = zi * A.z_alpha, hi = lo + A.z_alpha < A.nl ? lo + A.z_alpha : A.nl; return y >= lo && y < hi; }
    return y >= A.skip_lo && y < A.skip_hi;
}
__device__ __forceinline__ int hc_mm_mod(const HcMm &A, int y) { return y < A.nl ? y : A.nq + (y - A.nl); }
#define HC_MM_PROLOGUE \
    const int y = (int)blockIdx.y + ((int)blockIdx.y >= A.gap_lo ? A.gap_len : 0), zi = (int)blockIdx.z % A.nz, img = (int)blockIdx.z / A.nz; if (hc_mm_skip(A, y, zi)) return; \
    const HcRowMod R = hc_const_copy(&A.M[hc_mm_mod(A, y)]); \
    in += (size_t)zi * A.zs_in + (size_t)img * A.is_in; out += (size_t)zi * A.zs_out + (size_t)img * A.is_out;
#define HC_MM_PROLOGUE_ROWS \
    int bx, by_, bz_; \
    if (A.xcd) { const unsigned id = blockIdx.x, rest = id >> 3, p = (rest / (unsigned)A.nzn) * 8 + (id & 7); bx = (int)(p & 15); by_ = (int)(p >> 4); bz_ = (int)(rest % (unsigned)A.nzn); } \
    else { bx = (int)blockIdx.x; by_ = (int)blockIdx.y; bz_ = (int)blockIdx.z; } \
    const int y = by_ + (by_ >= A.gap_lo ? A.gap_len : 0), zi = bz_ % A.nz, img = bz_ / A.nz; if (hc_mm_skip(A, y, zi)) return; \
    const HcRowMod R = hc_const_copy(&A.M[hc_mm_mod(A, y)]); \
    in += (size_t)zi * A.zs_in + (size_t)img * A.is_in; out += (size_t)zi * A.zs_out + (size_t)img * A.is_out;
template <int EXT, int NS>
__device__ __forceinline__ void hc_cols_fwd_mm_small(const u64 *in, u64 *out, u32 *lds, const HcMm &A, const HcRowMod &R, int y, int zi, int img) {
    const int t = threadIdx.x, c = t & 15, tid = t >> 4;
    const u32 q = (u32)R.q;
    u32 e[16];
    if (EXT) {
        hc_basis_ext_tile32<NS>(e, in + blockIdx.x * 16 + c, hc_const_copy(&A.ext_bs[(A.z_alpha > 0 ? (size_t)zi * A.ext_rows : 0) + y]), tid);
        if (EXT == 2) {
            const u64 qL = A.mods[A.lift_level].q, h = (qL - 1) >> 1, qi = R.q, neg_h = qi - hc_barrett64(h, qi, R.mu);
            const u64 *tt = A.lift_t + (size_t)zi * A.lift_t_zs + (size_t)img * A.lift_t_is + blockIdx.x * 16 + c;
            const HcTw32 pm = hc_tw32(A.lift_pmul[y]);
#pragma unroll
            for (int hi = 0; hi < 16; hi++) {
                const u32 r = (u32)hc_barrett64(hc_csub(tt[(size_t)(hi * 16 + tid) * 256] + h, qL) + neg_h, qi, R.mu);
                e[hi] = hc_add32(e[hi], hc_mul32(r, pm, q), q);
// ... 901 lines not shown
```

### optimal_conv_amd/csrc/hconv.hip

```cpp
#ifdef HC_EMU
#include "hip_emu.h"
#else
#include <hip/hip_runtime.h>
#endif

#include <math.h>
#include <stdarg.h>
#include <stdio.h>
#include <string.h>

#include <map>
#include <utility>
#include <string>
#include <vector>

#include "../../include/hconv.h"
#include "../../include/hconv_test_hooks.h"
#include "hc_kernels.h"
#include "hc_gomath.h"
#ifndef HC_GX_LV
#define HC_GX_LV 64
#endif
#ifndef HC_GX_PW
#define HC_GX_PW 32
#endif
#ifndef HC_GX_YV
#define HC_GX_YV 256
#endif
#ifndef HC_GX_TEN
#define HC_GX_TEN 256
#endif
#ifndef HC_GX_LIN
#define HC_GX_LIN 128
#endif
#ifndef HC_GX_ROT
#define HC_GX_ROT 128
#endif
#ifndef HC_GX_QPMS
#define HC_GX_QPMS 256
#endif
#ifndef HC_GX_MAC
#define HC_GX_MAC 256
#endif
#ifndef HC_GX_MACM
#define HC_GX_MACM 256
#endif

#define HC_N 65536
#define HC_LOGN 16

static u64 h_mulmod(u64 a, u64 b, u64 q) { return (u64)(((u128)a * b) % q); }
static u64 h_powmod(u64 b, u64 e, u64 q) {
    u64 r = 1; b %= q;
    while (e) { if (e & 1) r = h_mulmod(r, b, q); b = h_mulmod(b, b, q); e >>= 1; }
    return r;
}
static u64 h_inv(u64 a, u64 q) { return h_powmod(a % q, q - 2, q); }
static u64 h_shoup(u64 w, u64 q) { return (u64)((((u128)w) << 64) / q); }
static HcTw h_pair(u64 w, u64 q) { HcTw p; p.w = w; p.ws = h_shoup(w, q); return p; }
static bool h_is_prime(u64 n) {
    if (n < 2) return false;
    for (u64 p : {2ull, 3ull, 5ull, 7ull, 11ull, 13ull, 17ull, 19ull, 23ull, 29ull, 31ull, 37ull}) { if (n % p == 0) return n == p; }
    u64 d = n - 1; int s = 0; while ((d & 1) == 0) { d >>= 1; s++; }
    for (u64 a : {2ull, 3ull, 5ull, 7ull, 11ull, 13ull, 17ull, 19ull, 23ull, 29ull, 31ull, 37ull}) {
        u64 x = h_powmod(a, d, n); if (x == 1 || x == n - 1) continue;
        bool comp = true;
        for (int i = 1; i < s; i++) { x = h_mulmod(x, x, n); if (x == n - 1) { comp = false; break; } }
        if (comp) return false;
    }
    return true;
}
static u64 h_primitive_root(u64 q) {
    std::vector<u64> fac; u64 n = q - 1;
    for (u64 p = 2; p * p <= n; p += (p == 2 ? 1 : 2)) if (n % p == 0) { fac.push_back(p); while (n % p == 0) n /= p; }
    if (n > 1) fac.push_back(n);
    for (u64 g = 3;; g++) {
        bool ok = true;
        for (u64 f : fac) if (h_powmod(g, (q - 1) / f, q) == 1) { ok = false; break; }
        if (ok) return g;
    }
}
static u32 h_bitrev16(u32 x) { u32 r = 0; for (int i = 0; i < 16; i++) { r = (r << 1) | (x & 1); x >>= 1; } return r; }

struct HcModHost {
    HcMod m;
    u64 psi, psi_inv;
    HcTwTab fwd, inv;
    HcTwTab32 fwd32 = {nullptr, nullptr, nullptr, nullptr}, inv32 = {nullptr, nullptr, nullptr, nullptr};
    HcTwTab inv_f64;
    std::vector<void *> allocs;
};
struct HcEvk { HcTw *q_rows; HcTw *p_rows; bool row_local; bool row256; };
struct HcSwk { u64 *rows = nullptr; int level = 0, beta = 0; };
struct HcProfRec { std::string name; hipEvent_t a, b; };
struct hc_ctx {
    int device = 0, nq = 0, np = 0;
    hipStream_t stream = nullptr;
    std::vector<HcModHost> mods;
    std::map<u64, HcEvk> evk;
    std::map<u64, HcSwk> swk;
    HcTw *idx_pairs = nullptr;
    u64 *ws_cts = nullptr; size_t ws_cts_rows = 0;
    u64 *ws_cts2 = nullptr; size_t ws_cts2_rows = 0;
    HcTw *ws_ctc = nullptr; size_t ws_ctc_cts = 0;
    u64 *ws_tmp = nullptr; size_t ws_tmp_rows = 0;
    HcMod *d_mods = nullptr; HcTw *d_csts = nullptr;
    struct CacheBlk { size_t n = 0; hipEvent_t ev = nullptr; bool pending = false; };
    std::map<char *, CacheBlk> cache_blk; std::map<size_t, std::vector<void *>> cache_free;
    int async_alloc = 0;
#ifdef HC_EMU
    long small_mm_wgs = 0;
#else
    long small_mm_wgs = 1024;
#endif
    long allocs_live = 0;
    HcRowMod *d_rowmods = nullptr;
    u64 *ws_mm = nullptr; size_t ws_mm_rows = 0;
    u64 *ws_accm = nullptr; size_t ws_accm_rows = 0;
    struct KsPlan { HcBasisExt *bx = nullptr, *bxdown = nullptr; HcTw *pinv = nullptr, *pmod = nullptr, *pinv_qlinv = nullptr, *yinv = nullptr, *yinv1 = nullptr; };
    std::map<int, KsPlan> ks_plan;
    std::map<int, HcTw *> rescale_plan;
    int nb = 1; size_t bs_poly = 0, bs_qp = 0;
    const void *hoist_cx = nullptr; int hoist_level = -1;
    long chunk_nodes = 64;
    hipEvent_t ev_fork = nullptr;
    HcCplx *enc_roots = nullptr; int *enc_rot_group = nullptr;
    hipEvent_t ev_shard = nullptr;
    u64 *ws_gather = nullptr; size_t ws_gather_rows = 0;
    long small_levels = 16;
    long peer_access = 1;
    int xcd_rows = 1;
    int pack32 = 1;
    int rot_fuse = 1;
    int small32 = 1;
    unsigned peer_warned = 0;
    unsigned peer_enabled = 0;
    long profile = 0;
    std::vector<HcProfRec> prof;
    std::map<std::string, std::pair<double, long>> prof_acc;
    hipEvent_t t0 = nullptr, t1 = nullptr;
    std::string err;
};
struct hc_ker { u64 *d = nullptr; int max_ob = 0; };

static std::string g_create_err;
static int hc_fail(hc_ctx *c, int code, const char *fmt, ...) {
    char buf[512]; va_list ap; va_start(ap, fmt); vsnprintf(buf, sizeof buf, fmt, ap); va_end(ap);
    if (c) c->err = buf; else g_create_err = buf;
    return code;
}
#define HC_HIP(c, call) do { hipError_t e_ = (call); if (e_ != hipSuccess) return hc_fail(c, HC_ERR_HIP, "%s: %s", #call, hipGetErrorString(e_)); } while (0)
#define HC_ENTER(c) do { if (!(c)) return HC_ERR_ARG; HC_HIP(c, hipSetDevice((c)->device)); } while (0)

static hipError_t hcx_malloc(hc_ctx *c, void **p, size_t n) {
    if (!(c && c->async_alloc)) return hipMalloc(p, n);
#ifndef HC_EMU
    if (c->async_alloc == 2) return hipMallocAsync(p, n, c->stream);
#endif
    auto it = c->cache_free.find(n);
    if (it != c->cache_free.end() && !it->second.empty()) { *p = it->second.back(); it->second.pop_back(); return hipSuccess; }
    hipError_t e = hipMalloc(p, n);
    if (e == hipSuccess) { hc_ctx::CacheBlk b; b.n = n; c->cache_blk[(char *)*p] = b; }
    return e;
}
static hipError_t hcx_free(hc_ctx *c, void *p) {
    if (!p) return hipSuccess;
    if (!(c && c->async_alloc)) return hipFree(p);
#ifndef HC_EMU
    if (c->async_alloc == 2) return hipFreeAsync(p, c->stream);
#endif
    auto it = c->cache_blk.find((char *)p);
    if (it == c->cache_blk.end()) return hipErrorInvalidDevicePointer;
    if (!it->second.ev && hipEventCreateWithFlags(&it->second.ev, hipEventDisableTiming) != hipSuccess) it->second.ev = nullptr;
    if (it->second.ev && hipEventRecord(it->second.ev, c->stream) == hipSuccess) it->second.pending = true;
    else { hipError_t e = hipStreamSynchronize(c->stream); if (e != hipSuccess) return e; it->second.pending = false; }
    c->cache_free[it->second.n].push_back(p);
    return hipSuccess;
}
static hipError_t hcx_h2d_async(hc_ctx *c, void *dst, const void *src, size_t n) {
    if (c->async_alloc && !c->cache_blk.empty()) {
        auto it = c->cache_blk.upper_bound((char *)dst);
        if (it != c->cache_blk.begin()) { --it; if ((char *)dst < it->first + it->second.n && it->second.pending) {
            hipError_t e = hipEventSynchronize(it->second.ev); if (e != hipSuccess) return e; it->second.pending = false; } }
    }
    return hipMemcpyAsync(dst, src, n, hipMemcpyHostToDevice, c->stream);
}
static hipError_t hcx_h2d(hc_ctx *c, void *dst, const void *src, size_t n) {
    hipError_t e = hcx_h2d_async(c, dst, src, n);
    return e != hipSuccess ? e : hipStreamSynchronize(c->stream);
}
struct HcScratch {
    hc_ctx *c; std::vector<void *> blocks;
    explicit HcScratch(hc_ctx *c_) : c(c_) {}
    ~HcScratch() { if (blocks.empty()) return; hipStreamSynchronize(c->stream); for (void *p : blocks) hcx_free(c, p); }
    template <class T> hipError_t alloc(T **p, size_t bytes) { *p = nullptr; hipError_t e = hcx_malloc(c, (void **)p, bytes); if (e == hipSuccess) blocks.push_back(*p); return e; }
    void keep(void *p) { for (auto it = blocks.begin(); it != blocks.end(); ++it) if (*it == p) { blocks.erase(it); return; } }
};
static inline bool hc_fm_free(u64 q) { return q < (1ull << 57); }
static inline bool hc_f64_ok(u64 q) { return q < (1ull << 49); }

template <int TPB = HC_TPB, class K, class... Args>
static int hc_launch(hc_ctx *c, const char *name, K kernel, dim3 grid, Args... args) {
    hipEvent_t a = nullptr, b = nullptr;
    if (c->profile) { HC_HIP(c, hipEventCreate(&a)); HC_HIP(c, hipEventCreate(&b)); HC_HIP(c, hipEventRecord(a, c->stream)); }
    hipLaunchKernelGGL(kernel, grid, dim3(TPB), 0, c->stream, args...);
    HC_HIP(c, hipGetLastError());
    if (c->profile) { HC_HIP(c, hipEventRecord(b, c->stream)); c->prof.push_back({name, a, b}); }
    return HC_OK;
}
#define HC_TRY(x) do { int r_ = (x); if (r_) return r_; } while (0)
static int hc_copy_d2d(hc_ctx *c, void *dst, const void *src, size_t bytes) {
    HC_HIP(c, hipMemcpyAsync(dst, src, bytes, hipMemcpyDeviceToDevice, c->stream));
    return HC_OK;
}
#define HC_LAUNCH_FM(q, c, name, KERNEL, grid, ...) \
    (hc_fm_free(q) ? hc_launch(c, name, KERNEL<HC_FM_FREE>, grid, __VA_ARGS__) : hc_launch(c, name, KERNEL<HC_FM_ALT>, grid, __VA_ARGS__))

static int hc_prof_flush(hc_ctx *c) {
    if (c->prof.empty()) return HC_OK;
    HC_HIP(c, hipStreamSynchronize(c->stream));
    for (auto &r : c->prof) {
        float ms = 0; HC_HIP(c, hipEventElapsedTime(&ms, r.a, r.b));
        auto &acc = c->prof_acc[r.name]; acc.first += ms; acc.second += 1;
        hipEventDestroy(r.a); hipEventDestroy(r.b);
    }
    c->prof.clear();
    return HC_OK;
}

template <class T>
static int hc_dev_upload(hc_ctx *c, HcModHost *owner, const std::vector<T> &v, const T **out) {
    void *d = nullptr;
    HC_HIP(c, hcx_malloc(c, &d, v.size() * sizeof(T)));
    HC_HIP(c, hcx_h2d(c, d, v.data(), v.size() * sizeof(T)));
    owner->allocs.push_back(d);
    *out = (const T *)d;
    return HC_OK;
}

static int hc_build_tables(hc_ctx *c, HcModHost *mh, bool inverse) {
    const u64 q = mh->m.q, base = inverse ? mh->psi_inv : mh->psi;
    std::vector<u64> pw(HC_N);
    {
        std::vector<u64> nat(HC_N); nat[0] = 1;
        for (int j = 1; j < HC_N; j++) nat[j] = h_mulmod(nat[j - 1], base, q);
        for (int j = 0; j < HC_N; j++) pw[h_bitrev16((u32)j)] = nat[j];
    }
    std::vector<HcTw> rowsA(256 * 16), rowsB((size_t)256 * 16 * 16), colsA(16), colsB(16 * 16);
    HcTw zero; zero.w = 0; zero.ws = 0;
    for (auto &x : rowsA) x = zero;
    for (auto &x : rowsB) x = zero;
    for (auto &x : colsA) x = zero;
    for (auto &x : colsB) x = zero;
    for (int s = 0; s < 4; s++) for (int g = 0; g < (1 << s); g++) {
// ... 396 lines not shown
    HC_TRY(hc_ensure_mm(c, (size_t)c->nb)); c->hoist_cx = nullptr;
    u64 *t = c->ws_mm;
    HC_TRY(hc_intt_mm(c, in_q0, t, 1, 1, 1, 0, 0, 0, 0, c->nb, c->bs_poly, (size_t)HC_N));
    HC_TRY(hc_launch(c, "mod_raise", hc_k_mod_raise, dim3(HC_GX_LV, (unsigned)(level + 1), (unsigned)c->nb), (const u64 *)t, (u64 *)out, (const HcMod *)c->d_mods, c->bs_poly));
    return hc_ntt_mm(c, out, out, level + 1, level + 1, 0, 0, 1, 0, 0, 0, c->nb, c->bs_poly, c->bs_poly);
}

extern "C" uint64_t hc_const_for(double constant, double q_level_f, uint64_t q, double *scale_mult) {
    double scale = 1.0;
    if (constant != 0) { double frac = constant - (double)(int64_t)constant; if (frac != 0) scale = q_level_f; }
    if (scale_mult) *scale_mult = scale;
    const bool neg = constant < 0;
    double x = (neg ? -scale * constant : scale * constant) + 0.5;
    u64 res;
    if (x < 18446744073709551616.0) res = (u64)x % q;
    else {
        int e; double mant = frexp(x, &e);
        u64 mi = (u64)ldexp(mant, 53); int sh = e - 53;
        u64 r = mi % q; for (int i = 0; i < sh; i++) { r += r; if (r >= q) r -= q; }
        res = r;
    }
    return neg ? q - res : res;
}

static dim3 hc_grid(int jobs, int z = 1) { return HC_JOB_FAST ? dim3((unsigned)jobs, 16, (unsigned)z) : dim3(16, (unsigned)jobs, (unsigned)z); }
static HcPtrs hc_ptrs1(const u64 *p) { HcPtrs P; memset(&P, 0, sizeof P); P.p[0] = p; return P; }
static int hc_fill_loopA(hc_ctx *c, HcLoopA *A, const HcPtrs &kers, u64 *cts, size_t cts_stride, int norm) {
    const HcModHost &m0 = c->mods[0], &m1 = c->mods[1];
    A->ctc = c->ws_ctc; A->ker = kers; A->tmp = c->ws_tmp; A->cts = cts; A->i0 = 0; A->norm = norm; A->slot0 = 0; A->slot_step = norm;
    A->cts_stride = cts_stride;
    A->m0 = m0.m; A->m1 = m1.m;
    A->q1inv = h_pair(h_inv(m1.m.q % m0.m.q, m0.m.q), m0.m.q);
    A->h = (m1.m.q - 1) >> 1; A->negh0 = m0.m.q - (A->h % m0.m.q);
    return HC_OK;
}

static int hc_ensure_ctc(hc_ctx *c, size_t nct) {
    if (c->ws_ctc_cts >= nct) return HC_OK;
    HC_HIP(c, hipStreamSynchronize(c->stream));
    if (c->ws_ctc) HC_HIP(c, hcx_free(c, c->ws_ctc));
    c->ws_ctc = nullptr; c->ws_ctc_cts = 0;
    HC_HIP(c, hcx_malloc(c, (void **)&c->ws_ctc, nct * 4 * HC_N * sizeof(HcTw)));
    c->ws_ctc_cts = nct;
    return HC_OK;
}
static int hc_prepare_ctc(hc_ctx *c, const HcPtrs &ct_in, int n, const u64 cst[2]) {
    HC_TRY(hc_ensure_ctc(c, (size_t)n));
    HcCtc K; K.m0 = c->mods[0].m; K.m1 = c->mods[1].m;
    K.c0 = h_pair(cst[0] % K.m0.q, K.m0.q); K.c1 = h_pair(cst[1] % K.m1.q, K.m1.q);
    return hc_launch(c, "ctc", hc_k_ctc_pairs, dim3(64, 4, (unsigned)n), ct_in, c->ws_ctc, K);
}

static int hc_loopA_run_set(hc_ctx *c, const HcPtrs &kers, int n, int i_first, int i_stride, int nch, u64 *cts, size_t cts_stride, bool compact) {
    long chunk = (c->chunk_nodes < 1 ? 1 : c->chunk_nodes) / n; if (chunk < 1) chunk = 1;
    if (chunk > nch) chunk = nch;
    HC_TRY(hc_ensure_tmp(c, (size_t)n * (size_t)chunk * 2));
    HcLoopA A; HC_TRY(hc_fill_loopA(c, &A, kers, cts, cts_stride, i_stride));
    const HcModHost &m0 = c->mods[0], &m1 = c->mods[1];
    for (int j0 = 0; j0 < nch; j0 += (int)chunk) {
        const int nj = (int)((nch - j0) < chunk ? (nch - j0) : chunk);
        A.i0 = i_first + j0 * i_stride;
        A.slot0 = compact ? j0 : A.i0; A.slot_step = compact ? 1 : i_stride;
        A.njobs = 2 * nj;
        const dim3 grid = hc_grid(2 * nj, n), flat = hc_grid(2 * nj * n);
        if (hc_f64_ok(m1.m.q)) {
            HC_TRY(hc_launch(c, "a1_mul_rowsinv", hc_k_a1<1>, grid, A, m1.inv_f64));
            HC_TRY(hc_fm_free(m0.m.q) ? hc_launch(c, "a2_colsinv_lift_colsfwd", hc_k_a2<HC_FM_FREE, 1>, flat, A, m1.inv_f64, m0.fwd)
                                      : hc_launch(c, "a2_colsinv_lift_colsfwd", hc_k_a2<HC_FM_ALT, 1>, flat, A, m1.inv_f64, m0.fwd));
        } else {
            HC_TRY(hc_launch(c, "a1_mul_rowsinv", hc_k_a1<0>, grid, A, m1.inv));
            HC_TRY(hc_fm_free(m0.m.q) ? hc_launch(c, "a2_colsinv_lift_colsfwd", hc_k_a2<HC_FM_FREE, 0>, flat, A, m1.inv, m0.fwd)
                                      : hc_launch(c, "a2_colsinv_lift_colsfwd", hc_k_a2<HC_FM_ALT, 0>, flat, A, m1.inv, m0.fwd));
        }
        HC_TRY(HC_LAUNCH_FM(m0.m.q, c, "a3_rowsfwd_rescale", hc_k_a3, grid, A, m0.fwd));
    }
    return HC_OK;
}
static int hc_loopA_run(hc_ctx *c, const u64 *ker, int max_ob, int norm, u64 *cts) {
    return hc_loopA_run_set(c, hc_ptrs1(ker), 1, 0, norm, max_ob / norm, cts, 0, false);
}

static int hc_rescale_plan(hc_ctx *c, int level, const HcTw **out) {
    auto it = c->rescale_plan.find(level);
    if (it == c->rescale_plan.end()) {
        const u64 qL = c->mods[(size_t)level].m.q;
        std::vector<HcTw> h((size_t)level);
        for (int i = 0; i < level; i++) { const u64 q = c->mods[(size_t)i].m.q; h[(size_t)i] = h_pair(h_inv(qL % q, q), q); }
        HcTw *d = nullptr; HC_HIP(c, hcx_malloc(c, (void **)&d, h.size() * sizeof(HcTw)));
        HC_HIP(c, hcx_h2d(c, d, h.data(), h.size() * sizeof(HcTw)));
        it = c->rescale_plan.emplace(level, d).first;
    }
    *out = it->second;
    return HC_OK;
}
static int hc_div_round_last_n(hc_ctx *c, int level, const u64 *x, size_t xs, u64 *out, size_t os, int np) {
    if (level < 1 || level >= c->nq) return hc_fail(c, HC_ERR_ARG, "hc_div_round_last: level %d outside 1..%d", level, c->nq - 1);
    if (!x || !out) return hc_fail(c, HC_ERR_ARG, "hc_div_round_last: null");
    HC_TRY(hc_batch_fits(c, "hc_div_round_last", level, false));
    if (level != 1) {
        const HcTw *qlinv; HC_TRY(hc_rescale_plan(c, level, &qlinv));
        const int nb = c->nb, nz = np * nb;
        HC_TRY(hc_ensure_mm(c, (size_t)nz * (level + 1)));
        c->hoist_cx = nullptr;
        u64 *t = c->ws_mm;
        HC_TRY(hc_intt_mm(c, x, t - (size_t)level * HC_N, level + 1, level + 1, np, xs, (size_t)HC_N, 0, level, nb, c->bs_poly, (size_t)np * HC_N, "rescale"));
        HcMmFuse F; F.lift_level = level; F.epi_x = x; F.epi_x_zs = xs; F.epi_x_is = c->bs_poly; F.epi_mul = qlinv;
        return hc_ntt_mm(c, t, out, level, level, 0, 0, np, (size_t)HC_N, os, 0, nb, (size_t)np * HC_N, c->bs_poly, "rescale", &F);
    }
    if (c->nb > 1) {
        const int nb = c->nb; const size_t bs = c->bs_poly; int rc = HC_OK;
        c->nb = 1;
        for (int g = 0; g < nb && !rc; g++) rc = hc_div_round_last_n(c, level, x + (size_t)g * bs, xs, out + (size_t)g * bs, os, np);
        c->nb = nb;
        return rc;
    }
    if (np != 1) { HC_TRY(hc_div_round_last_n(c, level, x, 0, out, 0, 1)); return hc_div_round_last_n(c, level, x + xs, 0, out + os, 0, 1); }
    HC_TRY(hc_ensure_tmp(c, 16));
    u64 *scratch = nullptr; HC_HIP(c, hcx_malloc(c, (void **)&scratch, (size_t)(2 + 4 + 4) * HC_N * sizeof(u64)));
    u64 *one = scratch, *cts = scratch + 2 * HC_N, *xx = scratch + 6 * HC_N;
    std::vector<u64> h((size_t)2 * HC_N, 1);
    int rc = HC_OK;
    if (hcx_h2d_async(c, one, h.data(), h.size() * sizeof(u64)) != hipSuccess || hipStreamSynchronize(c->stream) != hipSuccess
        || hipMemcpyAsync(xx, x, 2 * HC_N * sizeof(u64), hipMemcpyDeviceToDevice, c->stream) != hipSuccess
        || hipMemcpyAsync(xx + 2 * HC_N, x, 2 * HC_N * sizeof(u64), hipMemcpyDeviceToDevice, c->stream) != hipSuccess) rc = hc_fail(c, HC_ERR_HIP, "hc_div_round_last: staging copies failed");
    const u64 ones[2] = {1, 1};
    if (!rc) rc = hc_prepare_ctc(c, hc_ptrs1(xx), 1, ones);
    if (!rc) rc = hc_loopA_run(c, one, 1, 1, cts);
    if (!rc && hipMemcpyAsync(out, cts, HC_N * sizeof(u64), hipMemcpyDeviceToDevice, c->stream) != hipSuccess) rc = hc_fail(c, HC_ERR_HIP, "hc_div_round_last: result copy failed");
    if (hipStreamSynchronize(c->stream) != hipSuccess && !rc) rc = hc_fail(c, HC_ERR_HIP, "hc_div_round_last: stream synchronize failed");
    hcx_free(c, scratch);
    return rc;
}
extern "C" int hc_div_round_last(hc_ctx *c, int level, const uint64_t *x, uint64_t *out) { HC_ENTER(c); return hc_div_round_last_n(c, level, x, 0, out, 0, 1); }
extern "C" int hc_div_round_last2(hc_ctx *c, int level, const uint64_t *x0, const uint64_t *x1, uint64_t *out0, uint64_t *out1) {
    HC_ENTER(c);
    if (!x0 || !x1 || !out0 || !out1) return hc_fail(c, HC_ERR_ARG, "hc_div_round_last2: null");
    return hc_div_round_last_n(c, level, x0, (size_t)(x1 - x0), out0, (size_t)(out1 - out0), 2);
}

static bool hc_perm_row_local(u64 galEl, int top_bits = 4) {
    for (u32 i = 0; i < HC_N; i++) {
        u32 r = h_bitrev16(i), t = (u32)(((galEl * (2ull * r + 1)) & 0x1FFFF) >> 1), s = h_bitrev16(t);
        if ((s >> (16 - top_bits)) != (i >> (16 - top_bits))) return false;
    }
    return true;
}
extern "C" int hc_evk_load(hc_ctx *c, uint64_t galEl, const uint64_t *b_q, const uint64_t *a_q, const uint64_t *b_p, const uint64_t *a_p) {
    HC_ENTER(c);
    if (!b_q || !a_q || !b_p || !a_p || !(galEl & 1)) return hc_fail(c, HC_ERR_ARG, "hc_evk_load: bad arguments");
    if (c->np != 1) return hc_fail(c, HC_ERR_UNSUPPORTED, "hc_evk_load: level-0 key switching with one special prime (the pack evaluator of main.go:446-456) is what is implemented; np=%d", c->np);
    const HcModHost &m0 = c->mods[0], &mp = c->mods[(size_t)c->nq];
    HcScratch S(c);
    u64 *stage = nullptr; HC_HIP(c, S.alloc(&stage, 2 * HC_N * sizeof(u64)));
    HcEvk e; e.q_rows = nullptr; e.p_rows = nullptr; e.row_local = hc_perm_row_local(galEl); e.row256 = e.row_local && hc_perm_row_local(galEl, 8);
    u64 *stageq = nullptr; HC_HIP(c, S.alloc(&stageq, 2 * HC_N * sizeof(u64)));
    HC_HIP(c, S.alloc(&e.q_rows, 2 * HC_N * sizeof(HcTw)));
    HC_HIP(c, S.alloc(&e.p_rows, 2 * HC_N * sizeof(HcTw)));
    HC_HIP(c, hcx_h2d_async(c, stageq, b_q, HC_N * sizeof(u64)));
    HC_HIP(c, hcx_h2d_async(c, stageq + HC_N, a_q, HC_N * sizeof(u64)));
    HC_HIP(c, hcx_h2d_async(c, stage, b_p, HC_N * sizeof(u64)));
    HC_HIP(c, hcx_h2d_async(c, stage + HC_N, a_p, HC_N * sizeof(u64)));
    const HcTw pinv = h_pair(h_inv(mp.m.q % m0.m.q, m0.m.q), m0.m.q);
    HcTw z; z.w = z.ws = 0;
    int rc = hc_launch(c, "evk_from_mont", hc_k_pointwise<HC_PW_FROM_MONT>, hc_pw_grid(2 * HC_N), (const u64 *)stageq, (const u64 *)stageq, stageq, (size_t)2 * HC_N, m0.m, z);
    if (!rc) rc = hc_launch(c, "evk_div_p", hc_k_pointwise<HC_PW_MULC>, hc_pw_grid(2 * HC_N), (const u64 *)stageq, (const u64 *)stageq, stageq, (size_t)2 * HC_N, m0.m, pinv);
    if (!rc) rc = hc_launch(c, "make_pairs", hc_k_make_pairs, hc_pw_grid(2 * HC_N), (const u64 *)stageq, e.q_rows, (size_t)2 * HC_N, m0.m.q, 0);
    if (!rc) rc = hc_launch(c, "evk_from_mont", hc_k_pointwise<HC_PW_FROM_MONT>, hc_pw_grid(2 * HC_N), (const u64 *)stage, (const u64 *)stage, stage, (size_t)2 * HC_N, mp.m, z);
    if (!rc) rc = hc_launch(c, "evk_ninv", hc_k_pointwise<HC_PW_MULC>, hc_pw_grid(2 * HC_N), (const u64 *)stage, (const u64 *)stage, stage, (size_t)2 * HC_N, mp.m, h_pair(mp.m.ninv, mp.m.q));
    if (!rc) rc = hc_launch(c, "make_pairs", hc_k_make_pairs, hc_pw_grid(2 * HC_N), (const u64 *)stage, e.p_rows, (size_t)2 * HC_N, mp.m.q, 1);
    if (hipStreamSynchronize(c->stream) != hipSuccess && !rc) rc = hc_fail(c, HC_ERR_HIP, "hc_evk_load: stream synchronize failed");
    if (rc) return rc;
    S.keep(e.q_rows); S.keep(e.p_rows);
    auto it = c->evk.find(galEl);
    if (it != c->evk.end()) { hcx_free(c, it->second.q_rows); hcx_free(c, it->second.p_rows); }
    c->evk[galEl] = e;
    return HC_OK;
}

extern "C" int hc_idx_load(hc_ctx *c, const uint64_t *idx_host) {
    HC_ENTER(c);
    const HcModHost &m0 = c->mods[0];
    HcScratch S(c);
    u64 *stage = nullptr; HC_HIP(c, S.alloc(&stage, (size_t)HC_LOGN * HC_N * sizeof(u64)));
    if (idx_host) {
        HC_HIP(c, hcx_h2d_async(c, stage, idx_host, (size_t)HC_LOGN * HC_N * sizeof(u64)));
    } else {
        HC_HIP(c, hipMemsetAsync(stage, 0, (size_t)HC_LOGN * HC_N * sizeof(u64), c->stream));
        u64 one = 1;
        for (int i = 0; i < HC_LOGN; i++) HC_HIP(c, hcx_h2d_async(c, stage + (size_t)i * HC_N + ((size_t)1 << i), &one, sizeof one));
        HC_HIP(c, hipStreamSynchronize(c->stream));
        u64 *tmp = nullptr; HC_HIP(c, S.alloc(&tmp, (size_t)HC_LOGN * HC_N * sizeof(u64)));
        HC_TRY(HC_LAUNCH_FM(m0.m.q, c, "cols_fwd", hc_k_cols_fwd, dim3(16, HC_LOGN), (const u64 *)stage, tmp, m0.fwd, m0.m.q));
        HC_TRY(HC_LAUNCH_FM(m0.m.q, c, "rows_fwd_canon", hc_k_rows_fwd_canon, dim3(16, HC_LOGN), (const u64 *)tmp, stage, m0.fwd, m0.m.q, m0.m.mu));
    }
    HcTw *pairs = nullptr; HC_HIP(c, S.alloc(&pairs, (size_t)HC_LOGN * HC_N * sizeof(HcTw)));
    HC_TRY(hc_launch(c, "idx_pairs", hc_k_make_pairs, hc_pw_grid((size_t)HC_LOGN * HC_N), (const u64 *)stage, pairs, (size_t)HC_LOGN * HC_N, m0.m.q, 0));
    HC_HIP(c, hipStreamSynchronize(c->stream));
    S.keep(pairs);
    if (c->idx_pairs) HC_HIP(c, hcx_free(c, c->idx_pairs));
    c->idx_pairs = pairs;
    return HC_OK;
}

static int hc_ker_from_device(hc_ctx *c, u64 *d, int max_ob, bool take, hc_ker **out) {
    u64 *dst = d;
    int rc = HC_OK;
    if (!take) {
        HC_HIP(c, hcx_malloc(c, (void **)&dst, (size_t)max_ob * 2 * HC_N * sizeof(u64)));
        if (hipMemcpyAsync(dst, d, (size_t)max_ob * 2 * HC_N * sizeof(u64), hipMemcpyDeviceToDevice, c->stream) != hipSuccess) rc = hc_fail(c, HC_ERR_HIP, "hc_ker_load: device copy failed");
    }
    if (!rc && hipStreamSynchronize(c->stream) != hipSuccess) rc = hc_fail(c, HC_ERR_HIP, "hc_ker_load: stream synchronize failed");
    if (rc) { hcx_free(c, dst); return rc; }
    hc_ker *k = new hc_ker(); k->d = dst; k->max_ob = max_ob; *out = k;
    return HC_OK;
}
extern "C" int hc_ker_load(hc_ctx *c, const uint64_t *host, int max_ob, hc_ker **out) {
    HC_ENTER(c);
    if (!host || !out || max_ob < 1 || c->nq < 2) return hc_fail(c, HC_ERR_ARG, "hc_ker_load: bad arguments");
    HcScratch S(c);
    u64 *d = nullptr; HC_HIP(c, S.alloc(&d, (size_t)max_ob * 2 * HC_N * sizeof(u64)));
    HC_HIP(c, hcx_h2d_async(c, d, host, (size_t)max_ob * 2 * HC_N * sizeof(u64)));
    S.keep(d);
    return hc_ker_from_device(c, d, max_ob, true, out);
}
extern "C" int hc_ker_load_device(hc_ctx *c, const uint64_t *dptr, int max_ob, hc_ker **out) {
    HC_ENTER(c);
    if (!dptr || !out || max_ob < 1 || c->nq < 2) return hc_fail(c, HC_ERR_ARG, "hc_ker_load_device: bad arguments");
    return hc_ker_from_device(c, (u64 *)dptr, max_ob, false, out);
}
static int hc_prep_ker_impl(hc_ctx *c, const char *fn, const double *ker_in, int ker_len, const double *bn_a, int in_wid, int ker_wid,
                            int real_ib, int real_ob, int norm, double scale, int trans, int dil, int ib_stride, hc_ker **out) {
    if (!ker_in || !bn_a || !out || c->nq < 2 || in_wid < 1 || ker_wid < 1 || real_ib < 1 || real_ob < 1 || norm < 1 || (trans != 0 && trans != 1) ||
        dil < 1 || ib_stride < 1 || (trans && (dil != 1 || ib_stride != 1)))
        return hc_fail(c, HC_ERR_ARG, "%s: bad arguments", fn);
    if (HC_N % (in_wid * in_wid)) return hc_fail(c, HC_ERR_ARG, "%s: in_wid^2 must divide N", fn);
    const bool exp = dil != 1 || ib_stride != 1;
    const int max_bat = HC_N / (in_wid * in_wid), k_sz = ker_wid * ker_wid;
    if (ker_len != k_sz * real_ib * real_ob) return hc_fail(c, HC_ERR_ARG, "input size inconsistent!");
    const long kd = (long)dil * (ker_wid - 1) + 1;
    if ((long)norm * real_ib * ib_stride > max_bat || norm * real_ob > max_bat) return hc_fail(c, HC_ERR_ARG, "%s: norm*batch exceeds max_bat=%d", fn, max_bat);
    if (kd > in_wid) return hc_fail(c, HC_ERR_ARG, "%s: kernel too wide for this input width", fn);
    const int adj = (max_bat - 1) + max_bat * (in_wid + 1) * ((int)kd - 1) / 2;
    if (2 * adj > HC_N) return hc_fail(c, HC_ERR_ARG, "%s: kernel too wide for this input width", fn);
    HcScratch S(c);
    double *dk = nullptr, *da = nullptr; u64 *stage = nullptr, *dst = nullptr;
    HC_HIP(c, S.alloc(&dk, (size_t)ker_len * sizeof(double)));
    HC_HIP(c, S.alloc(&da, (size_t)real_ob * sizeof(double)));
    HC_HIP(c, S.alloc(&stage, (size_t)max_bat * 2 * HC_N * sizeof(u64)));
    HC_HIP(c, S.alloc(&dst, (size_t)max_bat * 2 * HC_N * sizeof(u64)));
    HC_HIP(c, hcx_h2d_async(c, dk, ker_in, (size_t)ker_len * sizeof(double)));
    HC_HIP(c, hcx_h2d_async(c, da, bn_a, (size_t)real_ob * sizeof(double)));
    HC_HIP(c, hipMemsetAsync(stage, 0, (size_t)max_bat * 2 * HC_N * sizeof(u64), c->stream));
    HcPrepKer P; P.ker_in = dk; P.bn_a = da; P.stage = stage; P.in_wid = in_wid; P.ker_wid = (int)kd; P.real_ib = real_ib; P.real_ob = real_ob;
    P.norm = norm; P.max_bat = max_bat; P.scale = scale; P.q0 = c->mods[0].m.q; P.q1 = c->mods[1].m.q;
    P.src_wid = ker_wid; P.dil = dil; P.ib_stride = ib_stride;
    int rc = exp ? hc_launch(c, "prep_ker_scatter_dilated", hc_k_prep_ker<false, true>, hc_pw_grid((size_t)ker_len), P)
           : trans ? hc_launch(c, "prep_ker_scatter_trans", hc_k_prep_ker<true>, hc_pw_grid((size_t)ker_len), P)
                   : hc_launch(c, "prep_ker_scatter", hc_k_prep_ker<false>, hc_pw_grid((size_t)ker_len), P);
    HC_HIP(c, hipStreamSynchronize(c->stream));
    for (int l = 0; l < 2 && !rc; l++) rc = hc_ntt(c, l, stage + (size_t)l * max_bat * HC_N, stage + (size_t)l * max_bat * HC_N, max_bat);
    if (!rc) rc = hc_launch(c, "ker_interleave", hc_k_ker_interleave, hc_pw_grid((size_t)max_bat * 2 * HC_N), (const u64 *)stage, dst, max_bat, c->mods[0].m, c->mods[1].m, 0);
    if (!rc && hipStreamSynchronize(c->stream) != hipSuccess) rc = hc_fail(c, HC_ERR_HIP, "%s: stream synchronize failed", fn);
    if (rc) return rc;
    S.keep(dst);
    hc_ker *k = new hc_ker(); k->d = dst; k->max_ob = max_bat; *out = k;
    return HC_OK;
}
extern "C" int hc_prep_ker_ex2(hc_ctx *c, const double *ker_in, int ker_len, const double *bn_a, int in_wid, int ker_wid,
                               int real_ib, int real_ob, int norm, double scale, int trans, int dilation, int ib_stride, hc_ker **out) {
    HC_ENTER(c);
    return hc_prep_ker_impl(c, "hc_prep_ker_ex2", ker_in, ker_len, bn_a, in_wid, ker_wid, real_ib, real_ob, norm, scale, trans, dilation, ib_stride, out);
}
extern "C" int hc_prep_ker_ex(hc_ctx *c, const double *ker_in, int ker_len, const double *bn_a, int in_wid, int ker_wid,
                              int real_ib, int real_ob, int norm, double scale, int trans, hc_ker **out) {
    HC_ENTER(c);
    return hc_prep_ker_impl(c, trans ? "hc_prep_ker_ex" : "hc_prep_ker", ker_in, ker_len, bn_a, in_wid, ker_wid, real_ib, real_ob, norm, scale, trans, 1, 1, out);
}
extern "C" int hc_prep_ker(hc_ctx *c, const double *ker_in, int ker_len, const double *bn_a, int in_wid, int ker_wid,
                           int real_ib, int real_ob, int norm, double scale, hc_ker **out) {
    return hc_prep_ker_ex(c, ker_in, ker_len, bn_a, in_wid, ker_wid, real_ib, real_ob, norm, scale, 0, out);
}
extern "C" int hc_ker_download(hc_ctx *c, const hc_ker *k, uint64_t *host_out) {
    HC_ENTER(c); if (!k || !host_out) return hc_fail(c, HC_ERR_ARG, "hc_ker_download: null");
    const size_t n = (size_t)k->max_ob * 2 * HC_N;
    HC_HIP(c, hipMemcpyAsync(host_out, k->d, n * sizeof(u64), hipMemcpyDeviceToHost, c->stream));
    HC_HIP(c, hipStreamSynchronize(c->stream));
    return HC_OK;
}
extern "C" void hc_ker_free(hc_ctx *c, hc_ker *k) { if (!k) return; if (c) { hipSetDevice(c->device); hipStreamSynchronize(c->stream); } hcx_free(c, k->d); delete k; }

static int hc_fill_loopB(hc_ctx *c, HcLoopB *B, const u64 *src, u64 *dst, const HcEvk &e, int logStep, int step, int norm, u64 galEl, int chunk) {
    const HcModHost &m0 = c->mods[0], &mp = c->mods[(size_t)c->nq];
    B->src = src; B->dst = dst;
    B->tmpC = c->ws_tmp; B->tmpE = c->ws_tmp + (size_t)chunk * HC_N; B->tmpT = c->ws_tmp + (size_t)chunk * 3 * HC_N;
    B->idx = c->idx_pairs + (size_t)logStep * HC_N;
    B->evkQ = e.q_rows; B->evkP = e.p_rows;
    B->n0 = 0; B->step = step; B->norm = norm; B->nodes = 1; B->src_stride = 0; B->dst_stride = 0;
    B->m0 = m0.m; B->mp = mp.m;
    B->pmodq = h_pair(mp.m.q % m0.m.q, m0.m.q);
    B->pinv = h_pair(h_inv(mp.m.q % m0.m.q, m0.m.q), m0.m.q);
    B->mu0 = (u64)((((u128)1) << 64) / m0.m.q);
    {
        const double pf = (double)mp.m.q;
        u64 lo = 0, hi = mp.m.q;
        while (lo < hi) { u64 mid = lo + (hi - lo) / 2; if ((u64)((double)mid / pf) >= 1) hi = mid; else lo = mid + 1; }
        B->vthresh = lo;
    }
    B->gal = (u32)(galEl & 0x1FFFF);
    return HC_OK;
}
static int hc_pack_level(hc_ctx *c, const u64 *src, u64 *dst, size_t sstride, size_t dstride, int n, int step, int logStep, int norm, u64 galEl, const HcPtrs *bias_last, const HcPtrs *outs_last = nullptr) {
    auto it = c->evk.find(galEl);
    if (it == c->evk.end()) return hc_fail(c, HC_ERR_STATE, "pack: no switching key loaded for galEl=%llu (the reference panics in permuteNTT)", (unsigned long long)galEl);
    if (!it->second.row_local) return hc_fail(c, HC_ERR_UNSUPPORTED, "pack: galEl=%llu does not permute inside 4096-coefficient tiles (needs max_cnum <= 4096)", (unsigned long long)galEl);
    if (!c->idx_pairs) HC_TRY(hc_idx_load(c, nullptr));
    const int nodes = (step + norm - 1) / norm;
    long chunkl = (c->chunk_nodes < 1 ? 1 : c->chunk_nodes) / n; if (chunkl < 1) chunkl = 1;
    const int chunk = (int)(chunkl < nodes ? chunkl : nodes);
    HC_TRY(hc_ensure_tmp(c, (size_t)n * chunk * 4));
    HcLoopB B; HC_TRY(hc_fill_loopB(c, &B, src, dst, it->second, logStep, step, norm, galEl, n * chunk));
    B.src_stride = sstride; B.dst_stride = dstride;
    if (it->second.row256) B.tmpT = nullptr;
    HcPtrs nobias; memset(&nobias, 0, sizeof nobias);
    const HcModHost &m0 = c->mods[0], &mp = c->mods[(size_t)c->nq];
    for (int n0 = 0; n0 < nodes; n0 += chunk) {
        const int nn = (nodes - n0) < chunk ? (nodes - n0) : chunk;
        B.n0 = n0; B.nodes = nn;
        const dim3 g1 = hc_grid(n * nn), g2 = hc_grid(2 * n * nn);
        if (c->small_levels > 0 && (long)n * nn <= c->small_levels && it->second.row256 && !HC_JOB_FAST) {
            const HcPtrs pb = bias_last ? *bias_last : nobias, po = outs_last ? *outs_last : nobias;
            B.tmpT = nullptr;
            const dim3 s1(HC_STILES, (unsigned)(n * nn)), s2(HC_STILES, (unsigned)(2 * n * nn)), s3(HC_STILES, (unsigned)(n * nn), 2);
            HC_TRY(hc_launch<HC_STPB>(c, "b1_node_rowsinv", hc_k_sb1, s1, B, m0.inv));
            HC_TRY(hc_launch<HC_STPB>(c, "b2_colsinv_colsfwdP", hc_k_sb2, s1, B, m0.inv, mp.fwd));
            HC_TRY(hc_launch<HC_STPB>(c, "b3_rowsfwdP_mac_rowsinvP", hc_k_sb3, s3, B, mp.fwd, mp.inv));
            HC_TRY(hc_launch<HC_STPB>(c, "b4_colsinvP_modup_colsfwd", hc_k_sb4, s2, B, mp.inv, m0.fwd));
            HC_TRY(hc_launch<HC_STPB>(c, "b5_rowsfwd_moddown_perm_add", hc_k_sb5, s2, B, m0.fwd, pb, po));
            continue;
        }
        HC_TRY(hc_launch(c, "b1_node_rowsinv", hc_k_b1, g1, B, m0.inv));
        HC_TRY(HC_LAUNCH_FM(mp.m.q, c, "b2_colsinv_colsfwdP", hc_k_b2, g1, B, m0.inv, mp.fwd));
        HC_TRY(HC_LAUNCH_FM(mp.m.q, c, "b3_rowsfwdP_mac_rowsinvP", hc_k_b3, g1, B, mp.fwd, mp.inv));
        HC_TRY(HC_LAUNCH_FM(m0.m.q, c, "b4_colsinvP_modup_colsfwd", hc_k_b4, g2, B, mp.inv, m0.fwd));
        const HcPtrs pb = bias_last ? *bias_last : nobias, po = outs_last ? *outs_last : nobias;
#if HC_B5M_LOADER && !defined(HC_EMU)
        if (it->second.row256) HC_TRY((hc_fm_free(m0.m.q) ? hc_launch<HC_LD_TPB>(c, "b5_rowsfwd_moddown_perm_add", hc_k_b5m_ld<HC_FM_FREE>, g1, B, m0.fwd, pb, po)
                                                          : hc_launch<HC_LD_TPB>(c, "b5_rowsfwd_moddown_perm_add", hc_k_b5m_ld<HC_FM_ALT>, g1, B, m0.fwd, pb, po)));
#else
        if (it->second.row256) HC_TRY(HC_LAUNCH_FM(m0.m.q, c, "b5_rowsfwd_moddown_perm_add", hc_k_b5m, g1, B, m0.fwd, pb, po));
#endif
        else HC_TRY(HC_LAUNCH_FM(m0.m.q, c, "b5_rowsfwd_moddown_perm_add", hc_k_b5, g2, B, m0.fwd, pb, po));
    }
    return HC_OK;
}
static int hc_pack_run(hc_ctx *c, u64 *cts, size_t cstride, int n, int max_cnum, int real_cnum, const HcPtrs *bias, int stride_log2 = 0, const HcPtrs *outs = nullptr) {
    if (max_cnum < 1 || real_cnum < 1 || max_cnum % real_cnum || (max_cnum & (max_cnum - 1)) || (real_cnum & (real_cnum - 1)))
        return hc_fail(c, HC_ERR_ARG, "pack: max_cnum=%d real_cnum=%d must be powers of two", max_cnum, real_cnum);
    const int norm = max_cnum / real_cnum;
    int step = max_cnum / 2, logStep = 0;
    for (int i = step; i > 1; i /= 2) logStep++;
    if (stride_log2 < 0 || logStep + stride_log2 >= HC_LOGN) return hc_fail(c, HC_ERR_ARG, "pack: stride_log2=%d out of range", stride_log2);
    int j = HC_LOGN - logStep - stride_log2;
    const size_t pong_one = (size_t)(max_cnum / 2 > 0 ? max_cnum / 2 : 1) * 2, pong_rows = pong_one * (size_t)n;
    if (c->ws_cts2_rows < pong_rows) {
        HC_HIP(c, hipStreamSynchronize(c->stream));
        if (c->ws_cts2) HC_HIP(c, hcx_free(c, c->ws_cts2));
        c->ws_cts2 = nullptr; c->ws_cts2_rows = 0;
        HC_HIP(c, hcx_malloc(c, (void **)&c->ws_cts2, pong_rows * HC_N * sizeof(u64)));
        c->ws_cts2_rows = pong_rows;
    }
    u64 *src = cts, *dst = c->ws_cts2;
    size_t sstride = cstride, dstride = pong_one * HC_N;
    bool bias_done = false, out_done = false;
    while (step >= norm && step >= 1) {
        const bool last = (step / 2 < norm) || step == 1;
        HC_TRY(hc_pack_level(c, src, dst, sstride, dstride, n, step, logStep + stride_log2, norm, (1ull << j) + 1, last ? bias : nullptr, last ? outs : nullptr));
        if (last) { bias_done = true; out_done = outs != nullptr; }
        u64 *t = src; src = dst; dst = t;
        size_t ts = sstride; sstride = dstride; dstride = ts;
        step /= 2; logStep--; j++;
    }
    if (out_done) return HC_OK;
    if (src != cts) for (int z = 0; z < n; z++)
        HC_TRY(hc_copy_d2d(c, cts + (size_t)z * cstride, src + (size_t)z * sstride, 2 * HC_N * sizeof(u64)));
    if (bias && !bias_done) {
        HcTw z0; z0.w = z0.ws = 0;
        for (int z = 0; z < n; z++) if (bias->p[z])
            HC_TRY(hc_launch(c, "bias_add", hc_k_pointwise<HC_PW_ADD>, hc_pw_grid(HC_N), (const u64 *)(cts + (size_t)z * cstride), bias->p[z], cts + (size_t)z * cstride, (size_t)HC_N, c->mods[0].m, z0));
    }
    if (outs) for (int z = 0; z < n; z++) HC_TRY(hc_copy_d2d(c, (void *)outs->p[z], cts + (size_t)z * cstride, 2 * HC_N * sizeof(u64)));
    return HC_OK;
}
extern "C" int hc_pack_ctxts(hc_ctx *c, uint64_t *cts, int max_cnum, int real_cnum) {
    HC_ENTER(c); if (!cts) return hc_fail(c, HC_ERR_ARG, "hc_pack_ctxts: null");
    return hc_pack_run(c, (u64 *)cts, 0, 1, max_cnum, real_cnum, nullptr);
}
extern "C" int hc_pack_ctxts_strided(hc_ctx *c, uint64_t *cts, int count, int stride_log2, const uint64_t *bias) {
    HC_ENTER(c); if (!cts) return hc_fail(c, HC_ERR_ARG, "hc_pack_ctxts_strided: null");
    const HcPtrs bp = hc_ptrs1((const u64 *)bias);
    return hc_pack_run(c, (u64 *)cts, 0, 1, count, count, bias ? &bp : nullptr, stride_log2);
}

extern "C" int hc_rotate_gal_l0(hc_ctx *c, uint64_t galEl, const uint64_t *c0, const uint64_t *c1, uint64_t *o0, uint64_t *o1);
static int hc_ks_common(hc_ctx *c, uint64_t galEl, const uint64_t *c0, const uint64_t *c1, uint64_t *o0, uint64_t *o1, bool rotate) {
    auto it = c->evk.find(galEl);
    if (it == c->evk.end()) return hc_fail(c, HC_ERR_STATE, "no switching key loaded for galEl=%llu", (unsigned long long)galEl);
    u64 *buf = nullptr; HC_HIP(c, hcx_malloc(c, (void **)&buf, (size_t)6 * HC_N * sizeof(u64)));
    u64 *y = buf, *x = buf + 2 * HC_N, *res = buf + 4 * HC_N;
    int rc = HC_OK;
    hipError_t he = hipMemsetAsync(x, 0, 2 * HC_N * sizeof(u64), c->stream);
    if (he == hipSuccess) he = c0 ? hipMemcpyAsync(y, c0, HC_N * sizeof(u64), hipMemcpyDeviceToDevice, c->stream) : hipMemsetAsync(y, 0, HC_N * sizeof(u64), c->stream);
    if (he == hipSuccess) he = hipMemcpyAsync(y + HC_N, c1, HC_N * sizeof(u64), hipMemcpyDeviceToDevice, c->stream);
    if (he != hipSuccess) rc = hc_fail(c, HC_ERR_HIP, "level-0 key switch: staging copies failed: %s", hipGetErrorString(he));
    if (!rc && !c->idx_pairs) rc = hc_idx_load(c, nullptr);
    const bool local = it->second.row_local;
    if (!rc) {
        if (rotate && local) {
            const int chunk = 1;
            rc = hc_ensure_tmp(c, 4);
            HcLoopB B; if (!rc) rc = hc_fill_loopB(c, &B, y, res, it->second, 0, 1, 1, galEl, chunk);
            const HcModHost &m0 = c->mods[0], &mp = c->mods[(size_t)c->nq];
            if (!rc) rc = hc_launch(c, "b1_node_rowsinv", hc_k_b1, hc_grid(1), B, m0.inv);
            if (!rc) rc = HC_LAUNCH_FM(mp.m.q, c, "b2_colsinv_colsfwdP", hc_k_b2, hc_grid(1), B, m0.inv, mp.fwd);
            if (!rc) rc = HC_LAUNCH_FM(mp.m.q, c, "b3_rowsfwdP_mac_rowsinvP", hc_k_b3, hc_grid(1), B, mp.fwd, mp.inv);
            if (!rc) rc = HC_LAUNCH_FM(m0.m.q, c, "b4_colsinvP_modup_colsfwd", hc_k_b4, hc_grid(2), B, mp.inv, m0.fwd);
            HcPtrs nobias; memset(&nobias, 0, sizeof nobias);
            if (!rc) rc = HC_LAUNCH_FM(m0.m.q, c, "b5_rowsfwd_moddown_perm_add", hc_k_b5, hc_grid(2), B, m0.fwd, nobias, nobias);
            HcTw z; z.w = z.ws = 0;
            if (!rc) rc = hc_launch(c, "ks_sub", hc_k_pointwise<HC_PW_SUB>, hc_pw_grid(2 * HC_N), (const u64 *)res, (const u64 *)y, res, (size_t)2 * HC_N, c->mods[0].m, z);
            if (!rc && (hipMemcpyAsync(o0, res, HC_N * sizeof(u64), hipMemcpyDeviceToDevice, c->stream) != hipSuccess
                        || hipMemcpyAsync(o1, res + HC_N, HC_N * sizeof(u64), hipMemcpyDeviceToDevice, c->stream) != hipSuccess)) rc = hc_fail(c, HC_ERR_HIP, "level-0 key switch: result copies failed");
        } else {
            rc = hc_fail(c, HC_ERR_UNSUPPORTED, "level-0 key switch is exposed for Galois elements that permute inside 4096-coefficient tiles (2^j+1, j>=5), the ones pack_ctxts uses");
        }
    }
    if (hipStreamSynchronize(c->stream) != hipSuccess && !rc) rc = hc_fail(c, HC_ERR_HIP, "level-0 key switch: stream synchronize failed");
    if (hcx_free(c, buf) != hipSuccess && !rc) rc = hc_fail(c, HC_ERR_HIP, "level-0 key switch: free failed");
    return rc;
}
extern "C" int hc_rotate_gal_l0(hc_ctx *c, uint64_t galEl, const uint64_t *c0, const uint64_t *c1, uint64_t *o0, uint64_t *o1) {
    HC_ENTER(c); if (!c0 || !c1 || !o0 || !o1) return hc_fail(c, HC_ERR_ARG, "hc_rotate_gal_l0: null");
    return hc_ks_common(c, galEl, c0, c1, o0, o1, true);
}
extern "C" int hc_keyswitch_l0(hc_ctx *c, uint64_t galEl, const uint64_t *c1, uint64_t *d0, uint64_t *d1) {
    HC_ENTER(c); if (!c1 || !d0 || !d1) return hc_fail(c, HC_ERR_ARG, "hc_keyswitch_l0: null");
    u64 *buf = nullptr; HC_HIP(c, hcx_malloc(c, (void **)&buf, (size_t)2 * HC_N * sizeof(u64)));
    int rc = hc_ks_common(c, galEl, nullptr, c1, buf, buf + HC_N, true);
    if (!rc) {
        u64 twoN = 2ull * HC_N, ginv = 1, b = galEl % twoN;
        for (u64 e = twoN - 1; e; e >>= 1, b = (b * b) % twoN) if (e & 1) ginv = (ginv * b) % twoN;
        rc = hc_permute(c, ginv, buf, d0, 1);
        if (!rc) rc = hc_permute(c, ginv, buf + HC_N, d1, 1);
    }
    hipStreamSynchronize(c->stream); hcx_free(c, buf);
    return rc;
}

static HcBasisExt hc_make_bx(const std::vector<u64> &src, u64 t) {
    HcBasisExt B; memset(&B, 0, sizeof B);
    B.n = (int)src.size(); B.t = t; B.mu_t = (u64)((((u128)1) << 64) / t);
    u64 smodt = 1;
    for (int i = 0; i < B.n; i++) {
        const u64 si = src[(size_t)i]; B.s[i] = si; B.mu_s[i] = (u64)((((u128)1) << 64) / si);
        u64 hat_si = 1, hat_t = 1;
        for (int j = 0; j < B.n; j++) if (j != i) { hat_si = h_mulmod(hat_si, src[(size_t)j] % si, si); hat_t = h_mulmod(hat_t, src[(size_t)j] % t, t); }
        B.inv[i] = h_pair(h_inv(hat_si, si), si);
        B.hat[i] = h_pair(hat_t, t);
        smodt = h_mulmod(smodt, si % t, t);
    }
    B.smodt = h_pair(smodt, t);
    return B;
}
extern "C" int hc_swk_load(hc_ctx *c, uint64_t key_id, int level, const uint64_t *rows_host) {
    HC_ENTER(c);
    if (!rows_host || level < 0 || level >= c->nq || c->np < 1 || c->np > HC_MAX_NP) return hc_fail(c, HC_ERR_ARG, "hc_swk_load: bad arguments");
    const int nt = level + 1 + c->np, beta = (level + 1 + c->np - 1) / c->np;
    const size_t n = (size_t)beta * 2 * nt * HC_N;
    HcSwk k; k.level = level; k.beta = beta;
    HC_HIP(c, hcx_malloc(c, (void **)&k.rows, n * sizeof(u64)));
    HC_HIP(c, hcx_h2d_async(c, k.rows, rows_host, n * sizeof(u64)));
    if (c->pack32) HC_TRY(hc_launch(c, "pack32_rows", hc_k_pack32_rows, dim3((unsigned)(beta * 2 * nt)), k.rows, (const HcMod *)c->d_mods, level + 1, c->nq, nt));
    HC_HIP(c, hipStreamSynchronize(c->stream));
    auto it = c->swk.find(key_id);
    if (it != c->swk.end()) hcx_free(c, it->second.rows);
    c->swk[key_id] = k;
    return HC_OK;
}
static int hc_swk_generate_impl(hc_ctx *c, uint64_t key_id, int level, uint64_t galEl, const uint64_t *sk_ntt, const uint32_t *seed8, bool splitmix, uint64_t sm_seed, const int64_t *e_host) {
    if (!sk_ntt || level < 0 || level >= c->nq || c->np < 1 || c->np > HC_MAX_NP || (galEl && !(galEl & 1))) return hc_fail(c, HC_ERR_ARG, "hc_swk_generate: bad arguments");
    const int alpha = c->np, nl = level + 1, nt = nl + alpha, beta = (nl + alpha - 1) / alpha;
    if (beta > 63 || nt > 62) return hc_fail(c, HC_ERR_UNSUPPORTED, "hc_swk_generate: more than 62 limbs");
    if (!splitmix && (key_id >> 40)) return hc_fail(c, HC_ERR_ARG, "hc_swk_generate: key id %llu does not fit the 40 bits of the ChaCha nonce that tell keys apart", (unsigned long long)key_id);
    HcKeyGen G; memset(&G, 0, sizeof G);
    if (seed8) memcpy(G.key, seed8, sizeof G.key);
    G.id_lo = (u32)key_id; G.id_hi = (u32)(key_id >> 32) & 0xFFu;
    G.relin = galEl == 0; G.nl = nl; G.nq = c->nq; G.nt = nt; G.alpha = alpha; G.beta = beta;
    if (galEl) { const u64 twoN = 2ull * HC_N; u64 ginv = 1, b = galEl % twoN; for (u64 e = twoN - 1; e; e >>= 1, b = (b * b) % twoN) if (e & 1) ginv = (ginv * b) % twoN; G.ginv = (u32)ginv; }
    const size_t n = (size_t)beta * 2 * nt * HC_N;
    HcScratch S(c);
    HcSwk k; k.level = level; k.beta = beta;
    HC_HIP(c, S.alloc(&k.rows, n * sizeof(u64)));
    HcTw *pm = nullptr; HC_HIP(c, S.alloc(&pm, (size_t)nl * sizeof(HcTw)));
    {   std::vector<HcTw> h((size_t)nl);
// ... 599 lines not shown
```

Before: 768.9 conv/s.

## Fuse both b5m components per block and use Montgomery-form idx/evk operands

The b5 moddown/permute/add kernel now processes both ciphertext components together in one pass, using a doubled LDS buffer and a paired rows-forward NTT, rather than looping over k. Index and key multipliers are stored as single Montgomery-form u64 words instead of 16-byte Shoup pairs, which halves that operand traffic and uses a lazy Montgomery multiply. Rows per batch go up and the wave hint drops. The unused async loader variant is removed. The costs are doubled LDS use and more registers per thread, which may lower occupancy, plus extra precompute buffers for the Montgomery tables.

```diff
diff --git a/optimal_conv_amd/csrc/hc_arith.h b/optimal_conv_amd/csrc/hc_arith.h
--- a/optimal_conv_amd/csrc/hc_arith.h
+++ b/optimal_conv_amd/csrc/hc_arith.h
@@ -82,6 +82,10 @@
     u64 r = hi - h;
     return hi < h ? r + q : r;
 }
+HC_HD u64 hc_mont_lazy(u64 x, u64 wm, u64 q, u64 qinv) {
+    const u128 m = (u128)x * wm;
+    return (u64)(m >> 64) + q - hc_mulhi((u64)m * qinv, q);
+}
 HC_HD u64 hc_mont_redc(u128 T, u64 q, u64 qinv) {
     const u64 lo = (u64)T, hi = (u64)(T >> 64);
     const u64 h = hc_mulhi(lo * qinv, q);
diff --git a/optimal_conv_amd/csrc/hc_kernels.h b/optimal_conv_amd/csrc/hc_kernels.h
--- a/optimal_conv_amd/csrc/hc_kernels.h
+++ b/optimal_conv_amd/csrc/hc_kernels.h
@@ -145,6 +145,9 @@
 template <bool KC = false> struct HcRowsTwA { const HcTw *p; __device__ __forceinline__ HcTw operator()(int slot) const { if (KC) return HC_TW_LOADK(p, slot); else return HC_TW_LOAD(p, slot); } };
 #ifndef HC_DBG_TWB_FIXED
 #define HC_DBG_TWB_FIXED 0
+#endif
+#if HC_DBG_TWB_FIXED
+#warning "HC_DBG_TWB_FIXED is set: a TIMING PROBE build - every residue that goes through a rows pass is WRONG"
 #endif
 template <bool KC = false> struct HcRowsTwB { const HcTw *p; __device__ __forceinline__ HcTw operator()(int slot) const { if (HC_DBG_TWB_FIXED) slot = 0; if (KC) return HC_TW_LOADK(p, slot * 16); else return HC_TW_LOAD(p, slot * 16); } };
 
@@ -841,6 +844,8 @@
     const HcTw *idx;
     const HcTw *evkQ;
     const HcTw *evkP;
+    const u64 *idxM;
+    const u64 *evkQM;
     int n0, step, norm;
     int nodes;
     size_t src_stride, dst_stride;
@@ -1015,268 +1020,108 @@
 }
 
 #ifndef HC_B5_ROWS
-#define HC_B5_ROWS 2
-#endif
-#ifndef HC_B5M_UNROLL
-#define HC_B5M_UNROLL 2
+#define HC_B5_ROWS 4
 #endif
 #ifndef HC_B5M_WAVES
-#define HC_B5M_WAVES 3
-#endif
-#ifndef HC_B5M_PIPE
-#define HC_B5M_PIPE 0
-#endif
-#define HC_PRAGMA_(x) _Pragma(#x)
-#define HC_UNROLL_N(n) HC_PRAGMA_(unroll n)
+#define HC_B5M_WAVES 2
+#endif
+template <int FM, class TW>
+__device__ __forceinline__ void hc_ct_round2(u64 (&e0)[16], u64 (&e1)[16], const TW &tw, const HcQ &Q) {
+#pragma unroll
+    for (int s = 0; s < 4; s++) {
+        const int half = 8 >> s;
+#pragma unroll
+        for (int g = 0; g < (1 << s); g++) {
+            const HcTw w = tw((1 << s) - 1 + g);
+#pragma unroll
+            for (int k = 0; k < half; k++) {
+                const int a = g * 2 * half + k, b = a + half;
+                u64 X0 = e0[a], X1 = e1[a];
+                if (FM == HC_FM_ALT) { X0 = hc_fold(X0, Q.nq4); X1 = hc_fold(X1, Q.nq4); }
+                const u64 T0 = hc_shoup4(e0[b], w.w, w.ws, Q), T1 = hc_shoup4(e1[b], w.w, w.ws, Q);
+                e0[a] = X0 + T0; e0[b] = (X0 + Q.q4) - T0;
+                e1[a] = X1 + T1; e1[b] = (X1 + Q.q4) - T1;
+            }
+        }
+    }
+}
+template <int FM>
+__device__ __forceinline__ void hc_rows_fwd2_lin(u64 (&e0)[16], u64 (&e1)[16], u64 *l0, u64 *l1, const HcTwTab &T, int row, int rloc, int tid, int t, const HcQ &Q) {
+    hc_ct_round2<FM>(e0, e1, HcRowsTwA<false>{T.rowsA + row * 16}, Q);
+#pragma unroll
+    for (int hi = 0; hi < 16; hi++) { const int a = hc_rows_lds(rloc, hi * 16 + tid); l0[a] = e0[hi]; l1[a] = e1[hi]; }
+    HC_ROW_SYNC();
+#pragma unroll
+    for (int lo = 0; lo < 16; lo++) { const int a = hc_rows_lds(rloc, tid * 16 + lo); e0[lo] = l0[a]; e1[lo] = l1[a]; }
+    hc_ct_round2<FM>(e0, e1, HcRowsTwB<false>{T.rowsB + row * 256 + tid}, Q);
+    HC_ROW_SYNC();
+#pragma unroll
+    for (int lo = 0; lo < 16; lo++) { const int a = hc_rows_lds(rloc, tid * 16 + lo); l0[a] = e0[lo]; l1[a] = e1[lo]; }
+    __syncthreads();
+#pragma unroll
+    for (int k = 0; k < 16; k++) { const int a = hc_rows_lds(k, t); e0[k] = l0[a]; e1[k] = l1[a]; }
+}
 template <int FM>
 __global__ __launch_bounds__(HC_TPB, HC_B5M_WAVES) void hc_k_b5m(HcLoopB B, HcTwTab T0fwd, HcPtrs biases, HcPtrs outs) {
-    __shared__ u64 lds[HC_ROWS_LDS];
+    __shared__ u64 lds[2 * HC_ROWS_LDS];
+    u64 *l0 = lds, *l1 = lds + HC_ROWS_LDS;
     const int t = threadIdx.x, tid = t & 15, rloc = t >> 4, row = HC_TILE * 16 + rloc;
     const int zn = HC_JOB, z = zn / B.nodes, node = zn - z * B.nodes, i = (B.n0 + node) * B.norm;
     const HcQ Q = hc_q(B.m0.q);
-    const u64 q = Q.q;
+    const u64 q = Q.q, qinv = B.m0.qinv;
     const size_t tile = (size_t)HC_TILE * 4096 + t;
     const u64 *__restrict__ ys = B.src + (size_t)z * B.src_stride + (size_t)i * 2 * 65536 + tile;
     const u64 *__restrict__ xs = B.src + (size_t)z * B.src_stride + (size_t)(i + B.step) * 2 * 65536 + tile;
-    const HcTw *__restrict__ idx = B.idx + tile;
-    const HcTw *__restrict__ evk = B.evkQ + tile;
+    const u64 *__restrict__ idx = B.idxM + tile;
+    const u64 *__restrict__ evk = B.evkQM + tile;
     u64 *__restrict__ o = (outs.p[z] != nullptr ? const_cast<u64 *>(outs.p[z]) : B.dst + (size_t)z * B.dst_stride + (size_t)i * 2 * 65536) + tile;
     const u64 *__restrict__ bias = biases.p[z] != nullptr ? biases.p[z] + tile : nullptr;
-    u64 e[16], T[16];
-#if HC_B5M_PIPE
-    HC_UNROLL_N(HC_B5M_UNROLL)
-    for (int k = 1; k >= 0; k--) {
-        const u64 *__restrict__ in = B.tmpE + ((size_t)zn * 2 + k) * 65536 + (size_t)row * 256;
-#pragma unroll
-        for (int hi = 0; hi < 16; hi++) e[hi] = in[hi * 16 + tid];
-        u64 Yn[HC_B5_ROWS], Xn[HC_B5_ROWS], bn[HC_B5_ROWS]; HcTw Kn[HC_B5_ROWS], In[HC_B5_ROWS];
+    u64 e0[16], e1[16];
+    {
+        const u64 *__restrict__ in = B.tmpE + (size_t)zn * 2 * 65536 + (size_t)row * 256;
+#pragma unroll
+        for (int hi = 0; hi < 16; hi++) { e0[hi] = in[hi * 16 + tid]; e1[hi] = in[65536 + hi * 16 + tid]; }
+    }
+    hc_rows_fwd2_lin<FM>(e0, e1, l0, l1, T0fwd, row, rloc, tid, t, Q);
+    __syncthreads();
+#pragma unroll
+    for (int b = 0; b < 16; b += HC_B5_ROWS) {
+        u64 Y0[HC_B5_ROWS], X0[HC_B5_ROWS], Y1[HC_B5_ROWS], X1[HC_B5_ROWS], K0[HC_B5_ROWS], K1[HC_B5_ROWS], I[HC_B5_ROWS], bs[HC_B5_ROWS], s0[HC_B5_ROWS], s1[HC_B5_ROWS];
 #pragma unroll
         for (int j = 0; j < HC_B5_ROWS; j++) {
-            const int off = j * 256;
-            Yn[j] = ys[(size_t)k * 65536 + off]; Xn[j] = xs[(size_t)k * 65536 + off]; In[j] = idx[off]; Kn[j] = evk[(size_t)k * 65536 + off];
-            bn[j] = (k == 0 && bias != nullptr) ? bias[off] : 0;
-        }
-        if (k == 0) __syncthreads();
-        hc_rows_fwd<FM>(e, lds, T0fwd, row, rloc, tid, Q);
-        HC_ROW_SYNC();
-        hc_rows_lo_to_lin(e, lds, t, rloc, tid);
+            const int off = (b + j) * 256;
+            Y1[j] = ys[65536 + off]; X1[j] = xs[65536 + off]; Y0[j] = ys[off]; X0[j] = xs[off]; I[j] = idx[off]; K0[j] = evk[off]; K1[j] = evk[65536 + off];
+            bs[j] = bias != nullptr ? bias[off] : 0;
+        }
+#pragma unroll
+        for (int j = 0; j < HC_B5_ROWS; j++) {
+            const int kk = b + j, a = hc_rows_lds(kk, t);
+            u64 m1 = hc_mont_lazy(X1[j], I[j], q, qinv), m0 = hc_mont_lazy(X0[j], I[j], q, qinv);
+            const u64 T = hc_fold(Y1[j] + Q.q4 - m1, Q.nq4);
+            u64 g1 = hc_mont_lazy(T, K1[j], q, qinv), g0 = hc_mont_lazy(T, K0[j], q, qinv);
+            if (FM == HC_FM_FREE) {
+                s1[j] = Y1[j] + m1; s0[j] = Y0[j] + m0 + bs[j];
+                l1[a] = g1 + HC_FREE_OFF * q - e1[kk];
+                l0[a] = Y0[j] + Q.q4 - m0 + g0 + HC_FREE_OFF * q - e0[kk];
+            } else {
+                m1 = hc_canon4(m1, Q); m0 = hc_canon4(m0, Q); g1 = hc_canon4(g1, Q); g0 = hc_canon4(g0, Q);
+                s1[j] = hc_addmod(Y1[j], m1, q); s0[j] = hc_addmod(hc_addmod(Y0[j], m0, q), bs[j], q);
+                l1[a] = hc_submod(g1, hc_canon8(e1[kk], Q), q);
+                l0[a] = hc_submod(hc_addmod(hc_submod(Y0[j], m0, q), g0, q), hc_canon8(e0[kk], Q), q);
+            }
+        }
         __syncthreads();
 #pragma unroll
-        for (int b = 0; b < 16; b += HC_B5_ROWS) {
-            u64 Y[HC_B5_ROWS], X[HC_B5_ROWS], t1[HC_B5_ROWS], bs[HC_B5_ROWS]; HcTw K[HC_B5_ROWS], I[HC_B5_ROWS];
-#pragma unroll
-            for (int j = 0; j < HC_B5_ROWS; j++) { Y[j] = Yn[j]; X[j] = Xn[j]; I[j] = In[j]; K[j] = Kn[j]; bs[j] = bn[j]; }
-            if (b + HC_B5_ROWS < 16) {
-#pragma unroll
-                for (int j = 0; j < HC_B5_ROWS; j++) {
-                    const int off = (b + HC_B5_ROWS + j) * 256;
-                    Yn[j] = ys[(size_t)k * 65536 + off]; Xn[j] = xs[(size_t)k * 65536 + off]; In[j] = idx[off]; Kn[j] = evk[(size_t)k * 65536 + off];
-                    bn[j] = (k == 0 && bias != nullptr) ? bias[off] : 0;
-                }
-            }
-#pragma unroll
-            for (int j = 0; j < HC_B5_ROWS; j++) {
-                const int kk = b + j;
-                u64 m = hc_shoup4(X[j], I[j].w, I[j].ws, Q), f;
-                if (k == 1) T[kk] = hc_fold(Y[j] + Q.q4 - m, Q.nq4);
-                u64 g = hc_shoup4(T[kk], K[j].w, K[j].ws, Q);
-                if (FM == HC_FM_FREE) {
-                    t1[j] = Y[j] + m + bs[j];
-                    f = (k == 0 ? Y[j] + Q.q4 - m + g : g) + HC_FREE_OFF * q - e[kk];
-                } else {
-                    m = hc_canon4(m, Q); g = hc_canon4(g, Q);
-                    t1[j] = hc_addmod(hc_addmod(Y[j], m, q), bs[j], q);
-                    f = hc_submod(k == 0 ? hc_addmod(hc_submod(Y[j], m, q), g, q) : g, hc_canon8(e[kk], Q), q);
-                }
-                lds[hc_rows_lds(kk, t)] = f;
-            }
-            __syncthreads();
-#pragma unroll
-            for (int j = 0; j < HC_B5_ROWS; j++) {
-                const int kk = b + j;
-                const u32 srcidx = hc_perm_src((u32)((HC_TILE * 16 + kk) * 256 + t), B.gal);
-                const u64 d = lds[hc_rows_lds(kk, (int)(srcidx & 255))];
-                o[(size_t)k * 65536 + kk * 256] = FM == HC_FM_FREE ? hc_reduce64(t1[j] + d, B.m0.mu, Q) : hc_addmod(t1[j], d, q);
-            }
-        }
-    }
-#else
-    HC_UNROLL_N(HC_B5M_UNROLL)
-    for (int k = 1; k >= 0; k--) {
-        const u64 *__restrict__ in = B.tmpE + ((size_t)zn * 2 + k) * 65536 + (size_t)row * 256;
-#pragma unroll
-        for (int hi = 0; hi < 16; hi++) e[hi] = in[hi * 16 + tid];
-        if (k == 0) __syncthreads();
-        hc_rows_fwd<FM>(e, lds, T0fwd, row, rloc, tid, Q);
-        HC_ROW_SYNC();
-        hc_rows_lo_to_lin(e, lds, t, rloc, tid);
-        __syncthreads();
-#pragma unroll
-        for (int b = 0; b < 16; b += HC_B5_ROWS) {
-            u64 Y[HC_B5_ROWS], X[HC_B5_ROWS], t1[HC_B5_ROWS], bs[HC_B5_ROWS]; HcTw K[HC_B5_ROWS], I[HC_B5_ROWS];
-#pragma unroll
-            for (int j = 0; j < HC_B5_ROWS; j++) {
-                const int off = (b + j) * 256;
-                Y[j] = ys[(size_t)k * 65536 + off]; X[j] = xs[(size_t)k * 65536 + off]; I[j] = idx[off]; K[j] = evk[(size_t)k * 65536 + off];
-                bs[j] = (k == 0 && bias != nullptr) ? bias[off] : 0;
-            }
-#pragma unroll
-            for (int j = 0; j < HC_B5_ROWS; j++) {
-                const int kk = b + j;
-                u64 m = hc_shoup4(X[j], I[j].w, I[j].ws, Q), f;
-                if (k == 1) T[kk] = hc_fold(Y[j] + Q.q4 - m, Q.nq4);
-                u64 g = hc_shoup4(T[kk], K[j].w, K[j].ws, Q);
-                if (FM == HC_FM_FREE) {
-                    t1[j] = Y[j] + m + bs[j];
-                    f = (k == 0 ? Y[j] + Q.q4 - m + g : g) + HC_FREE_OFF * q - e[kk];
-                } else {
-                    m = hc_canon4(m, Q); g = hc_canon4(g, Q);
-                    t1[j] = hc_addmod(hc_addmod(Y[j], m, q), bs[j], q);
-                    f = hc_submod(k == 0 ? hc_addmod(hc_submod(Y[j], m, q), g, q) : g, hc_canon8(e[kk], Q), q);
-                }
-                lds[hc_rows_lds(kk, t)] = f;
-            }
-            __syncthreads();
-#pragma unroll
-            for (int j = 0; j < HC_B5_ROWS; j++) {
-                const int kk = b + j;
-                const u32 srcidx = hc_perm_src((u32)((HC_TILE * 16 + kk) * 256 + t), B.gal);
-                const u64 d = lds[hc_rows_lds(kk, (int)(srcidx & 255))];
-                o[(size_t)k * 65536 + kk * 256] = FM == HC_FM_FREE ? hc_reduce64(t1[j] + d, B.m0.mu, Q) : hc_addmod(t1[j], d, q);
-            }
-        }
-    }
-#endif
-}
-
-#ifndef HC_B5M_LOADER
-#define HC_B5M_LOADER 0
-#endif
-#if HC_B5M_LOADER && !defined(HC_EMU)
-#ifndef HC_LD_RING
-#define HC_LD_RING 4
-#endif
-#ifndef HC_LD_AUX
-#define HC_LD_AUX 0
-#endif
-#define HC_LD_SLOT 1536
-#define HC_LD_TPB (HC_TPB + 64)
-typedef const void __attribute__((address_space(1))) *HcGlobalVoidPtr;
-typedef void __attribute__((address_space(3))) *HcLdsVoidPtr;
-__device__ __forceinline__ void hc_wait_vmcnt(int n) {
-#define HC_VMC(k) case k: asm volatile("s_waitcnt vmcnt(" #k ")" ::: "memory"); break;
-    switch (n) { HC_VMC(0) HC_VMC(12) HC_VMC(24) HC_VMC(36) HC_VMC(48) HC_VMC(60) default: asm volatile("s_waitcnt vmcnt(0)" ::: "memory"); break; }
-#undef HC_VMC
-}
-__device__ __forceinline__ void hc_ld_row(u64 *ring, int slot, const u64 *ys, const u64 *xs, const HcTw *idx, const HcTw *evk, int k, int kk, int lane) {
-    u64 *s = ring + slot * HC_LD_SLOT;
-    const u64 *y = ys + (size_t)k * 65536 + kk * 256 + lane * 2, *x = xs + (size_t)k * 65536 + kk * 256 + lane * 2;
-    const HcTw *I = idx + kk * 256 + lane, *K = evk + (size_t)k * 65536 + kk * 256 + lane;
-#pragma unroll
-    for (int h = 0; h < 2; h++) {
-        __builtin_amdgcn_global_load_lds((HcGlobalVoidPtr)(y + h * 128), (HcLdsVoidPtr)(s + h * 128), 16, 0, HC_LD_AUX);
-        __builtin_amdgcn_global_load_lds((HcGlobalVoidPtr)(x + h * 128), (HcLdsVoidPtr)(s + 256 + h * 128), 16, 0, HC_LD_AUX);
-    }
-#pragma unroll
-    for (int h = 0; h < 4; h++) {
-        __builtin_amdgcn_global_load_lds((HcGlobalVoidPtr)(I + h * 64), (HcLdsVoidPtr)(s + 512 + h * 128), 16, 0, 0);
-        __builtin_amdgcn_global_load_lds((HcGlobalVoidPtr)(K + h * 64), (HcLdsVoidPtr)(s + 1024 + h * 128), 16, 0, 0);
-    }
-}
-__device__ __forceinline__ void hc_ld_rows(int g0, int g1, u64 *ring, const u64 *ys, const u64 *xs, const HcTw *idx, const HcTw *evk, int lane) {
-#pragma unroll
-    for (int g = g0; g < g1; g++)
-        if (g < 32) hc_ld_row(ring, g % HC_LD_RING, ys, xs, idx, evk, g < 16 ? 1 : 0, g & 15, lane);
-}
-constexpr int hc_ld_min(int a, int b) { return a < b ? a : b; }
-template <int FM>
-__global__ __launch_bounds__(HC_LD_TPB, 3) void hc_k_b5m_ld(HcLoopB B, HcTwTab T0fwd, HcPtrs biases, HcPtrs outs) {
-    __shared__ u64 lds[HC_ROWS_LDS + HC_LD_RING * HC_LD_SLOT];
-    u64 *ring = lds + HC_ROWS_LDS;
-    constexpr int R = HC_B5_ROWS, S = HC_LD_RING, NBAT = 16 / R;
-    static_assert(S >= 2 * R && S % R == 0 && (S - R) * 12 <= 60, "ring: at least two row batches, a whole number of them, and a vmcnt that fits its 6-bit field");
-    const int zn = HC_JOB, z = zn / B.nodes, node = zn - z * B.nodes, i = (B.n0 + node) * B.norm;
-    const size_t tile0 = (size_t)HC_TILE * 4096;
-    const u64 *__restrict__ ys0 = B.src + (size_t)z * B.src_stride + (size_t)i * 2 * 65536 + tile0;
-    const u64 *__restrict__ xs0 = B.src + (size_t)z * B.src_stride + (size_t)(i + B.step) * 2 * 65536 + tile0;
-    if (threadIdx.x >= HC_TPB) {
-        const int lane = threadIdx.x - HC_TPB;
-        const HcTw *idx0 = B.idx + tile0, *evk0 = B.evkQ + tile0;
-        hc_ld_rows(0, S, ring, ys0, xs0, idx0, evk0, lane);
-#pragma unroll
-        for (int k = 1; k >= 0; k--) {
-            const int gb0 = (1 - k) * NBAT;
-            if (k == 0) __builtin_amdgcn_s_barrier();
-            __builtin_amdgcn_s_barrier();
-            hc_wait_vmcnt((hc_ld_min(gb0 * R + S, 32) - (gb0 + 1) * R) * 12);
-            __builtin_amdgcn_s_barrier();
-#pragma unroll
-            for (int b = 0; b < NBAT; b++) {
-                const int gb = gb0 + b, left = hc_ld_min(gb * R + S, 32) - (gb + 2) * R;
-                if (b + 1 < NBAT) hc_wait_vmcnt(left < 0 ? 0 : left * 12);
-                __builtin_amdgcn_s_barrier();
-                hc_ld_rows(gb * R + S, gb * R + S + R, ring, ys0, xs0, idx0, evk0, lane);
-            }
-        }
-        return;
-    }
-    const int t = threadIdx.x, tid = t & 15, rloc = t >> 4, row = HC_TILE * 16 + rloc;
-    const HcQ Q = hc_q(B.m0.q);
-    const u64 q = Q.q;
-    u64 *__restrict__ o = (outs.p[z] != nullptr ? const_cast<u64 *>(outs.p[z]) : B.dst + (size_t)z * B.dst_stride + (size_t)i * 2 * 65536) + tile0 + t;
-    const u64 *__restrict__ bias = biases.p[z] != nullptr ? biases.p[z] + tile0 + t : nullptr;
-    u64 e[16], T[16];
-    HC_UNROLL_N(HC_B5M_UNROLL)
-    for (int k = 1; k >= 0; k--) {
-        const u64 *__restrict__ in = B.tmpE + ((size_t)zn * 2 + k) * 65536 + (size_t)row * 256;
-#pragma unroll
-        for (int hi = 0; hi < 16; hi++) e[hi] = in[hi * 16 + tid];
-        if (k == 0) __syncthreads();
-        hc_rows_fwd<FM>(e, lds, T0fwd, row, rloc, tid, Q);
-        HC_ROW_SYNC();
-        hc_rows_lo_to_lin(e, lds, t, rloc, tid);
-        __syncthreads();
-        auto epilogue = [&](auto HB) {
-            constexpr bool HASB = decltype(HB)::value;
-#pragma unroll
-            for (int b = 0; b < 16; b += R) {
-                u64 Y[R], X[R], t1[R], bs[R]; HcTw K[R], I[R];
-#pragma unroll
-                for (int j = 0; j < R; j++) {
-                    const u64 *s = ring + (((1 - k) * 16 + b + j) % S) * HC_LD_SLOT;
-                    Y[j] = s[t]; X[j] = s[256 + t]; I[j] = *reinterpret_cast<const HcTw *>(s + 512 + 2 * t); K[j] = *reinterpret_cast<const HcTw *>(s + 1024 + 2 * t);
-                    bs[j] = HASB ? bias[(b + j) * 256] : 0;
-                }
-#pragma unroll
-                for (int j = 0; j < R; j++) {
-                    const int kk = b + j;
-                    u64 m = hc_shoup4(X[j], I[j].w, I[j].ws, Q), f;
-                    if (k == 1) T[kk] = hc_fold(Y[j] + Q.q4 - m, Q.nq4);
-                    u64 g = hc_shoup4(T[kk], K[j].w, K[j].ws, Q);
-                    if (FM == HC_FM_FREE) {
-                        t1[j] = Y[j] + m + bs[j];
-                        f = (k == 0 ? Y[j] + Q.q4 - m + g : g) + HC_FREE_OFF * q - e[kk];
-                    } else {
-                        m = hc_canon4(m, Q); g = hc_canon4(g, Q);
-                        t1[j] = hc_addmod(hc_addmod(Y[j], m, q), bs[j], q);
-                        f = hc_submod(k == 0 ? hc_addmod(hc_submod(Y[j], m, q), g, q) : g, hc_canon8(e[kk], Q), q);
-                    }
-                    lds[hc_rows_lds(kk, t)] = f;
-                }
-                __syncthreads();
-#pragma unroll
-                for (int j = 0; j < R; j++) {
-                    const int kk = b + j;
-                    const u32 srcidx = hc_perm_src((u32)((HC_TILE * 16 + kk) * 256 + t), B.gal);
-                    const u64 d = lds[hc_rows_lds(kk, (int)(srcidx & 255))];
-                    o[(size_t)k * 65536 + kk * 256] = FM == HC_FM_FREE ? hc_reduce64(t1[j] + d, B.m0.mu, Q) : hc_addmod(t1[j], d, q);
-                }
-            }
-        };
-        if (k == 0 && bias != nullptr) epilogue(HcBool<true>{}); else epilogue(HcBool<false>{});
-    }
-}
-#endif
+        for (int j = 0; j < HC_B5_ROWS; j++) {
+            const int kk = b + j;
+            const u32 srcidx = hc_perm_src((u32)((HC_TILE * 16 + kk) * 256 + t), B.gal);
+            const int a = hc_rows_lds(kk, (int)(srcidx & 255));
+            const u64 d1 = l1[a], d0 = l0[a];
+            o[65536 + kk * 256] = FM == HC_FM_FREE ? hc_reduce64(s1[j] + d1, B.m0.mu, Q) : hc_addmod(s1[j], d1, q);
+            o[kk * 256] = FM == HC_FM_FREE ? hc_reduce64(s0[j] + d0, B.m0.mu, Q) : hc_addmod(s0[j], d0, q);
+        }
+    }
+}
 
 #define HC_STPB 256
 #define HC_STILES 64
@@ -1602,6 +1447,9 @@
 #endif
 #ifndef HC_DBG_EXT_ONELOAD
 #define HC_DBG_EXT_ONELOAD 0
+#endif
+#if HC_DBG_EXT_ONELOAD
+#warning "HC_DBG_EXT_ONELOAD is set: a TIMING PROBE build - the basis extensions compute WRONG residues"
 #endif
 #define HC_MAX_NP 5
 template <int NS>
diff --git a/optimal_conv_amd/csrc/hconv.hip b/optimal_conv_amd/csrc/hconv.hip
--- a/optimal_conv_amd/csrc/hconv.hip
+++ b/optimal_conv_amd/csrc/hconv.hip
@@ -90,7 +90,7 @@
     HcTwTab inv_f64;
     std::vector<void *> allocs;
 };
-struct HcEvk { HcTw *q_rows; HcTw *p_rows; bool row_local; bool row256; };
+struct HcEvk { HcTw *q_rows; HcTw *p_rows; u64 *q_mont; bool row_local; bool row256; };
 struct HcSwk { u64 *rows = nullptr; int level = 0, beta = 0; };
 struct HcProfRec { std::string name; hipEvent_t a, b; };
 struct hc_ctx {
@@ -100,6 +100,7 @@
     std::map<u64, HcEvk> evk;
     std::map<u64, HcSwk> swk;
     HcTw *idx_pairs = nullptr;
+    u64 *idx_mont = nullptr;
     u64 *ws_cts = nullptr; size_t ws_cts_rows = 0;
     u64 *ws_cts2 = nullptr; size_t ws_cts2_rows = 0;
     HcTw *ws_ctc = nullptr; size_t ws_ctc_cts = 0;
@@ -802,9 +803,10 @@
     const HcModHost &m0 = c->mods[0], &mp = c->mods[(size_t)c->nq];
     HcScratch S(c);
     u64 *stage = nullptr; HC_HIP(c, S.alloc(&stage, 2 * HC_N * sizeof(u64)));
-    HcEvk e; e.q_rows = nullptr; e.p_rows = nullptr; e.row_local = hc_perm_row_local(galEl); e.row256 = e.row_local && hc_perm_row_local(galEl, 8);
+    HcEvk e; e.q_rows = nullptr; e.p_rows = nullptr; e.q_mont = nullptr; e.row_local = hc_perm_row_local(galEl); e.row256 = e.row_local && hc_perm_row_local(galEl, 8);
     u64 *stageq = nullptr; HC_HIP(c, S.alloc(&stageq, 2 * HC_N * sizeof(u64)));
-    HC_HIP(c, S.alloc(&e.q_rows, 2 * HC_N * sizeof(HcTw)));
+    HC_HIP(c, S.alloc(&e.q_rows, 2 * HC_N * (sizeof(HcTw) + sizeof(u64))));
+    e.q_mont = reinterpret_cast<u64 *>(e.q_rows + 2 * HC_N);
     HC_HIP(c, S.alloc(&e.p_rows, 2 * HC_N * sizeof(HcTw)));
     HC_HIP(c, hcx_h2d_async(c, stageq, b_q, HC_N * sizeof(u64)));
     HC_HIP(c, hcx_h2d_async(c, stageq + HC_N, a_q, HC_N * sizeof(u64)));
@@ -815,6 +817,7 @@
     int rc = hc_launch(c, "evk_from_mont", hc_k_pointwise<HC_PW_FROM_MONT>, hc_pw_grid(2 * HC_N), (const u64 *)stageq, (const u64 *)stageq, stageq, (size_t)2 * HC_N, m0.m, z);
     if (!rc) rc = hc_launch(c, "evk_div_p", hc_k_pointwise<HC_PW_MULC>, hc_pw_grid(2 * HC_N), (const u64 *)stageq, (const u64 *)stageq, stageq, (size_t)2 * HC_N, m0.m, pinv);
     if (!rc) rc = hc_launch(c, "make_pairs", hc_k_make_pairs, hc_pw_grid(2 * HC_N), (const u64 *)stageq, e.q_rows, (size_t)2 * HC_N, m0.m.q, 0);
+    if (!rc) rc = hc_launch(c, "evk_to_mont", hc_k_pointwise<HC_PW_TO_MONT>, hc_pw_grid(2 * HC_N), (const u64 *)stageq, (const u64 *)stageq, e.q_mont, (size_t)2 * HC_N, m0.m, z);
     if (!rc) rc = hc_launch(c, "evk_from_mont", hc_k_pointwise<HC_PW_FROM_MONT>, hc_pw_grid(2 * HC_N), (const u64 *)stage, (const u64 *)stage, stage, (size_t)2 * HC_N, mp.m, z);
     if (!rc) rc = hc_launch(c, "evk_ninv", hc_k_pointwise<HC_PW_MULC>, hc_pw_grid(2 * HC_N), (const u64 *)stage, (const u64 *)stage, stage, (size_t)2 * HC_N, mp.m, h_pair(mp.m.ninv, mp.m.q));
     if (!rc) rc = hc_launch(c, "make_pairs", hc_k_make_pairs, hc_pw_grid(2 * HC_N), (const u64 *)stage, e.p_rows, (size_t)2 * HC_N, mp.m.q, 1);
@@ -843,12 +846,15 @@
         HC_TRY(HC_LAUNCH_FM(m0.m.q, c, "cols_fwd", hc_k_cols_fwd, dim3(16, HC_LOGN), (const u64 *)stage, tmp, m0.fwd, m0.m.q));
         HC_TRY(HC_LAUNCH_FM(m0.m.q, c, "rows_fwd_canon", hc_k_rows_fwd_canon, dim3(16, HC_LOGN), (const u64 *)tmp, stage, m0.fwd, m0.m.q, m0.m.mu));
     }
-    HcTw *pairs = nullptr; HC_HIP(c, S.alloc(&pairs, (size_t)HC_LOGN * HC_N * sizeof(HcTw)));
+    HcTw *pairs = nullptr; HC_HIP(c, S.alloc(&pairs, (size_t)HC_LOGN * HC_N * (sizeof(HcTw) + sizeof(u64))));
+    u64 *mont = reinterpret_cast<u64 *>(pairs + (size_t)HC_LOGN * HC_N);
+    HcTw z; z.w = z.ws = 0;
     HC_TRY(hc_launch(c, "idx_pairs", hc_k_make_pairs, hc_pw_grid((size_t)HC_LOGN * HC_N), (const u64 *)stage, pairs, (size_t)HC_LOGN * HC_N, m0.m.q, 0));
+    HC_TRY(hc_launch(c, "idx_to_mont", hc_k_pointwise<HC_PW_TO_MONT>, hc_pw_grid((size_t)HC_LOGN * HC_N), (const u64 *)stage, (const u64 *)stage, mont, (size_t)HC_LOGN * HC_N, m0.m, z));
     HC_HIP(c, hipStreamSynchronize(c->stream));
     S.keep(pairs);
     if (c->idx_pairs) HC_HIP(c, hcx_free(c, c->idx_pairs));
-    c->idx_pairs = pairs;
+    c->idx_pairs = pairs; c->idx_mont = mont;
     return HC_OK;
 }
 
@@ -945,6 +951,7 @@
     B->tmpC = c->ws_tmp; B->tmpE = c->ws_tmp + (size_t)chunk * HC_N; B->tmpT = c->ws_tmp + (size_t)chunk * 3 * HC_N;
     B->idx = c->idx_pairs + (size_t)logStep * HC_N;
     B->evkQ = e.q_rows; B->evkP = e.p_rows;
+    B->idxM = c->idx_mont + (size_t)logStep * HC_N; B->evkQM = e.q_mont;
     B->n0 = 0; B->step = step; B->norm = norm; B->nodes = 1; B->src_stride = 0; B->dst_stride = 0;
     B->m0 = m0.m; B->mp = mp.m;
     B->pmodq = h_pair(mp.m.q % m0.m.q, m0.m.q);
@@ -993,12 +1000,7 @@
         HC_TRY(HC_LAUNCH_FM(mp.m.q, c, "b3_rowsfwdP_mac_rowsinvP", hc_k_b3, g1, B, mp.fwd, mp.inv));
         HC_TRY(HC_LAUNCH_FM(m0.m.q, c, "b4_colsinvP_modup_colsfwd", hc_k_b4, g2, B, mp.inv, m0.fwd));
         const HcPtrs pb = bias_last ? *bias_last : nobias, po = outs_last ? *outs_last : nobias;
-#if HC_B5M_LOADER && !defined(HC_EMU)
-        if (it->second.row256) HC_TRY((hc_fm_free(m0.m.q) ? hc_launch<HC_LD_TPB>(c, "b5_rowsfwd_moddown_perm_add", hc_k_b5m_ld<HC_FM_FREE>, g1, B, m0.fwd, pb, po)
-                                                          : hc_launch<HC_LD_TPB>(c, "b5_rowsfwd_moddown_perm_add", hc_k_b5m_ld<HC_FM_ALT>, g1, B, m0.fwd, pb, po)));
-#else
         if (it->second.row256) HC_TRY(HC_LAUNCH_FM(m0.m.q, c, "b5_rowsfwd_moddown_perm_add", hc_k_b5m, g1, B, m0.fwd, pb, po));
-#endif
         else HC_TRY(HC_LAUNCH_FM(m0.m.q, c, "b5_rowsfwd_moddown_perm_add", hc_k_b5, g2, B, m0.fwd, pb, po));
     }
     return HC_OK;
```

After: 784.2 conv/s (median of 6 runs). 2.0% higher.
